# truemeat001/Simple-Raytracing-Render

Measured on AMD Instinct MI355X. Metric: Msamples/s (rays x bounces) + HBM GB/s vs roofline, Cornell+teapot 1024spp, higher is better.
Workload: dtype f32

## Files before the change

### simple-raytracing-render_amd/csrc/capi.cpp

```cpp
#include <hip/hip_runtime.h>

#include <algorithm>
#include <chrono>
#include <cstdint>
#include <cstdio>
#include <cstring>
#include <map>
#include <memory>
#include <string>
#include <vector>

#include "../../include/srr_capi.h"
#include "imageio.h"
#include "meshio.h"
#include "../../include/srr/merl.h"
#include "multi.h"
#include "renderer.h"

using namespace srr;

struct srr_scene {
  Scene s;
};

namespace {
thread_local std::string g_err;

int fail(int code, const std::string& msg) {
  g_err = msg;
  return code;
}

#define HIPCHK(x)                                                                         \
  do {                                                                                    \
    hipError_t e_ = (x);                                                                  \
    if (e_ != hipSuccess) return fail(SRR_EIO, std::string(#x) + ": " + hipGetErrorString(e_)); \
  } while (0)

template <class T>
int upload(T** dst, const std::vector<T>& v) {
  size_t bytes = std::max<size_t>(v.size() * sizeof(T), 16);
  HIPCHK(hipMalloc((void**)dst, bytes));
  if (!v.empty()) HIPCHK(hipMemcpy(*dst, v.data(), v.size() * sizeof(T), hipMemcpyHostToDevice));
  return 0;
}
}

extern "C" {

const char* srr_last_error(void) { return g_err.c_str(); }
const char* srr_version(void) { return "srr 0.1 (gfx950 wavefront path tracer)"; }

srr_scene* srr_scene_create(void) { return new srr_scene(); }
void srr_scene_destroy(srr_scene* s) { delete s; }

int srr_scene_from_text(const char* text, srr_scene** out) {
  if (!text || !out) return fail(SRR_EINVAL, "null argument");
  std::unique_ptr<srr_scene> s(new srr_scene());
  std::string err;
  int rc = scene_from_text(text, s->s, err);
  if (rc < 0) return fail(rc, err);
  *out = s.release();
  return 0;
}

int srr_scene_text_handle(const srr_scene* s, int id) {
  if (!s) return fail(SRR_EINVAL, "null scene");
  for (auto& kv : s->s.text_ids)
    if (kv.first == id) return kv.second;
  return fail(SRR_EINVAL, "no such text object id");
}

int srr_scene_digest(const srr_scene* s, uint64_t* out, uint64_t* parts) {
  if (!s || !out) return fail(SRR_EINVAL, "null argument");
  Flat f;
  std::string err;
  const int rc = flatten(s->s, f, err);
  if (rc < 0) return fail(rc, err);
  uint64_t h = 0xcbf29ce484222325ULL;
  int part = 0;
  auto mix = [](uint64_t& x, const void* p, size_t n) {
    const unsigned char* b = (const unsigned char*)p;
    for (size_t i = 0; i < n; ++i) x = (x ^ b[i]) * 0x100000001b3ULL;
  };
  auto blob = [&](const void* p, size_t n) {
    mix(h, &n, sizeof n);
    mix(h, p, n);
    if (const char* dd = getenv("SRR_DIGEST_DUMP")) {
      FILE* df = fopen((std::string(dd) + "." + std::to_string(part)).c_str(), "wb");
      if (df) { fwrite(p, 1, n, df); fclose(df); }
    }
    if (parts) {
      uint64_t x = 0xcbf29ce484222325ULL;
      mix(x, p, n);
      parts[part] = x;
    }
    ++part;
  };
  auto vec = [&blob](const auto& v) { blob(v.data(), v.size() * sizeof(v[0])); };
  vec(f.objs);
  blob(&f.n_world, sizeof f.n_world);
  vec(f.xforms);
  vec(f.spheres);
  vec(f.rects);
  vec(f.stris);
  vec(f.meshes);
  vec(f.nodes);
  vec(f.node4);
  vec(f.tri_pos);
  vec(f.tri_shade);
  vec(f.media);
  {
    std::vector<uint8_t> b;
    auto put = [&b](const void* p, size_t n) { b.insert(b.end(), (const uint8_t*)p, (const uint8_t*)p + n); };
    put(f.obvhs.data(), f.obvhs.size() * sizeof(DObvh));
    put(f.sgroups.data(), f.sgroups.size() * sizeof(DSGroup));
    put(f.sg_items.data(), f.sg_items.size() * sizeof(DSGItem));
    vec(b);
  }
  vec(f.obvh_children);
  vec(f.mats);
  vec(f.texs);
  vec(f.images);
  vec(f.perlin_ranvec);
  vec(f.perlin_perm);
  vec(f.lights);
  blob(&f.cam, sizeof f.cam);
  *out = h;
  return 0;
}

int srr_scene_set_lcg(srr_scene* s, uint64_t state) {
  if (!s) return fail(SRR_EINVAL, "null scene");
  s->s.lcg = state & 0xFFFFFFFFFFFFULL;
  return 0;
}
uint64_t srr_scene_get_lcg(const srr_scene* s) { return s ? s->s.lcg : 0; }
double srr_scene_drand48(srr_scene* s) { return s ? s->s.drand48() : 0.0; }

#define SCN(s) \
  if (!(s)) return fail(SRR_EINVAL, "null scene");
#define TEXOK(s, t) \
  if (!(s)->s.valid_tex(t)) return fail(SRR_EINVAL, "bad texture handle " + std::to_string(t));
#define MATOK(s, m) \
  if (!(s)->s.valid_mat(m)) return fail(SRR_EINVAL, "bad material handle " + std::to_string(m));
#define OBJOK(s, o) \
  if (!(s)->s.valid_obj(o)) return fail(SRR_EINVAL, "bad hitable handle " + std::to_string(o));

int srr_constant_texture(srr_scene* s, float r, float g, float b) {
  SCN(s);
  HTex t;
  t.kind = TEX_CONST;
  t.c[0] = r; t.c[1] = g; t.c[2] = b;
  return s->s.add_tex(std::move(t));
}
int srr_image_texture(srr_scene* s, const unsigned char* rgb, int nx, int ny) {
  SCN(s);
  if (!rgb || nx <= 0 || ny <= 0) return fail(SRR_EINVAL, "bad image");
  HTex t;
  t.kind = TEX_IMAGE;
  t.nx = nx;
  t.ny = ny;
  t.px.assign(rgb, rgb + (size_t)nx * ny * 3);
  return s->s.add_tex(std::move(t));
}
int srr_image_texture_file(srr_scene* s, const char* path) {
  SCN(s);
  if (!path) return fail(SRR_EINVAL, "null path");
  srr::Image im;
  std::string err;
// ... 301 lines not shown
    hipError_t e = hipMemcpy(h.data(), d, h.size() * sizeof(float), hipMemcpyDeviceToHost);
    if (e != hipSuccess) rc = fail(SRR_EIO, hipGetErrorString(e));
  }
  hipFree(d);
  if (rc < 0) return rc;
  if (mean) std::memcpy(mean, h.data(), h.size() * sizeof(float));
  if (rgb8) srr_tonemap(h.data(), npix, rgb8);
  return 0;
}

int srr_accum_get(srr_renderer* r, float* sums, int64_t* npix, int64_t* samples) {
  if (!r) return fail(SRR_EINVAL, "null renderer");
  if (r && r->multi) return fail(SRR_EINVAL, "progressive sums and kept paths are per device: use a one-device renderer");
  if (npix) *npix = r->acc_npix;
  if (samples) *samples = r->acc_samples;
  if (sums && r->acc_npix) {
    HIPCHK(hipSetDevice(r->device));
    HIPCHK(hipMemcpy(sums, r->acc, 3 * r->acc_npix * sizeof(float), hipMemcpyDeviceToHost));
  }
  return 0;
}

int srr_accum_set(srr_renderer* r, const float* sums, int64_t npix, int64_t samples) {
  if (!r || !sums || npix <= 0 || samples < 0) return fail(SRR_EINVAL, "bad accumulator state");
  if (r && r->multi) return fail(SRR_EINVAL, "progressive sums and kept paths are per device: use a one-device renderer");
  HIPCHK(hipSetDevice(r->device));
  drain_async(r);
  if ((size_t)npix > r->pix_cap) {
    r->pix_key[0] = -1;
    (void)hipFree(r->pixels);
    (void)hipFree(r->acc);
    r->pixels = nullptr;
    r->acc = nullptr;
    r->pix_cap = 0;
    HIPCHK(hipMalloc((void**)&r->pixels, npix * sizeof(int32_t)));
    HIPCHK(hipMalloc((void**)&r->acc, 3 * npix * sizeof(float)));
    r->pix_cap = npix;
  }
  HIPCHK(hipMemcpy(r->acc, sums, 3 * npix * sizeof(float), hipMemcpyHostToDevice));
  r->acc_npix = npix;
  r->acc_samples = samples;
  std::fill(r->acc_key, r->acc_key + 5, -1);
  return 0;
}

int srr_copy_paths(srr_renderer* r, float* radiance, unsigned char* rays) {
  if (r && r->multi) return fail(SRR_EINVAL, "progressive sums and kept paths are per device: use a one-device renderer");
  if (!r || !r->raw_all) return fail(SRR_EINVAL, "render with SRR_FLAG_KEEP_PATHS first");
  HIPCHK(hipSetDevice(r->device));
  if (radiance) HIPCHK(hipMemcpy(radiance, r->raw_all, r->kept_paths * 3 * sizeof(float), hipMemcpyDeviceToHost));
  if (rays) HIPCHK(hipMemcpy(rays, r->rays_all, r->kept_paths, hipMemcpyDeviceToHost));
  return 0;
}

int srr_tonemap(const float* mean, int64_t n, unsigned char* rgb8) {
  if (!mean || !rgb8) return fail(SRR_EINVAL, "null argument");
  for (int64_t i = 0; i < 3 * n; ++i) {
    float c = std::sqrt(mean[i]);
    int q = int(255.99 * c);
    q = q > 255 ? 255 : q;
    q = q < 0 ? 0 : q;
    rgb8[i] = (unsigned char)q;
  }
  return 0;
}

int srr_mesh_file_triangles(const char* path, int flip_uvs, int flip_winding, const float scale[3], float* pos9,
                            float* uv9, float* nrm9, int* flags_out) {
  if (!path || !scale) return fail(SRR_EINVAL, "null argument");
  srr::MeshData m;
  std::string err;
  if (srr::load_mesh_file(path, m, err) < 0) return fail(SRR_EIO, err);
  srr::apply_model_semantics(m, flip_uvs != 0, flip_winding != 0, scale);
  for (size_t t = 0; t < m.tris.size(); ++t)
    for (int j = 0; j < 3; ++j) {
      const srr::MeshData::Corner& c = m.tris[t][j];
      if (pos9) std::memcpy(pos9 + 9 * t + 3 * j, c.p, 12);
      if (uv9) std::memcpy(uv9 + 9 * t + 3 * j, c.uv, 12);
      if (nrm9) std::memcpy(nrm9 + 9 * t + 3 * j, c.n, 12);
    }
  if (flags_out) *flags_out = (m.has_normals ? 1 : 0) | (m.has_uvs ? 2 : 0);
  if (m.tris.size() > (size_t)INT32_MAX / 2) return fail(SRR_EINVAL, "mesh too large");
  return (int)m.tris.size();
}

int srr_model(srr_scene* s, const char* path, int flip_uvs, int flip_winding, int mat, const float scale[3],
              int* first_handle) {
  if (!s || !path || !scale) return fail(SRR_EINVAL, "null argument");
  srr::MeshData m;
  std::string err;
  if (srr::load_mesh_file(path, m, err) < 0) return fail(SRR_EIO, err);
  srr::apply_model_semantics(m, flip_uvs != 0, flip_winding != 0, scale);
  if (m.tris.empty()) return fail(SRR_EINVAL, std::string(path) + ": mesh 0 has no triangles");
  int first = -1;
  for (const auto& t : m.tris) {
    float p[9], uv[9], n[9];
    for (int j = 0; j < 3; ++j) {
      std::memcpy(p + 3 * j, t[j].p, 12);
      std::memcpy(uv + 3 * j, t[j].uv, 12);
      std::memcpy(n + 3 * j, t[j].n, 12);
    }
    int h = srr_triangle(s, p, mat, uv, m.has_normals ? n : nullptr);
    if (h < 0) return h;
    if (first < 0) first = h;
  }
  if (first_handle) *first_handle = first;
  return (int)m.tris.size();
}

int srr_write_ppm(const char* path, int nx, int ny, const unsigned char* rgb8) {
  FILE* f = fopen(path, "w");
  if (!f) return fail(SRR_EIO, std::string("cannot open ") + path);
  fprintf(f, "P3\n%d %d\n255\n", nx, ny);
  for (int i = 0; i < nx * ny; ++i) fprintf(f, "%d %d %d\n", rgb8[3 * i], rgb8[3 * i + 1], rgb8[3 * i + 2]);
  fclose(f);
  return 0;
}

int srr_write_png(const char* path, int nx, int ny, const unsigned char* rgb8) {
  if (!path || !rgb8) return fail(SRR_EINVAL, "null argument");
  std::vector<uint8_t> png;
  std::string err;
  int rc = srr::encode_png(rgb8, nx, ny, 3, png, err);
  if (rc < 0) return fail(rc, err);
  FILE* f = fopen(path, "wb");
  if (!f) return fail(SRR_EIO, std::string("cannot open ") + path);
  size_t w = fwrite(png.data(), 1, png.size(), f);
  fclose(f);
  return w == png.size() ? 0 : fail(SRR_EIO, std::string("short write to ") + path);
}

int srr_image_load(const char* path, int req_comp, int* x, int* y, int* comp, unsigned char** out) {
  if (!path || !x || !y || !out) return fail(SRR_EINVAL, "null argument");
  *out = nullptr;
  srr::Image im;
  std::string err;
  int rc = srr::load_image(path, req_comp, im, err);
  if (rc < 0) return fail(rc == -2 ? SRR_EIO : SRR_EINVAL, err);
  *x = im.w;
  *y = im.h;
  if (comp) *comp = im.file_n;
  *out = (unsigned char*)malloc(im.px.size());
  if (!*out) return fail(SRR_ENOMEM, "out of memory");
  std::memcpy(*out, im.px.data(), im.px.size());
  return im.n;
}

void srr_image_free(unsigned char* pixels) { free(pixels); }

int srr_device_kat(const char* name, int n, int width, float* records) {
  if (!name || !records || n <= 0 || width <= 0) return fail(SRR_EINVAL, "bad KAT arguments");
  static const char* kNames[] = {"erf",   "beckmann11", "beckmann_dist", "beckmann_pdf", "cosine_pdf",
                                 "orennayar_pdf", "dielectric", "metal", "triangle", "aabb", "sqrt",
                                 "camera", "lights", "light_list"};
  static const int kWidth[] = {3, 5, 16, 21, 21, 21, 14, 14, 26, 15, 2, 23, 15, 15};
  int kind = -1;
  for (int k = 0; k < 14; ++k)
    if (!strcmp(name, kNames[k])) kind = k;
  if (kind < 0) return fail(SRR_EINVAL, std::string("no device KAT named ") + name);
  if (width != kWidth[kind]) return fail(SRR_EINVAL, std::string("KAT ") + name + ": unexpected record width");
  std::vector<float> aux(4 * (size_t)n, 0.f);
  std::vector<DStandaloneTri> tris(kind == 8 ? n : 1);
  Scene hs;
  for (int q = 0; q < n; ++q) {
    const float* r = records + (size_t)q * width;
    if (kind == 2 || kind == 3) {
      const float prm[4] = {r[0], r[1], 0, 0};
      const HMat& m = hs.mat[hs.material(MAT_BECKMANN, -1, prm)];
      aux[4 * q] = m.p[0];
      aux[4 * q + 1] = m.p[1];
    } else if (kind == 4 || kind == 5) {
      const float prm[4] = {r[0], 0, 0, 0};
      const HMat& m = hs.mat[hs.material(MAT_ORENNAYAR, -1, prm)];
      aux[4 * q] = m.p[0];
      aux[4 * q + 1] = m.p[1];
    } else if (kind == 8) {
      const float uv9[9] = {0.1f, 0.2f, 0, 0.7f, 0.1f, 0, 0.3f, 0.9f, 0};
      const int h = hs.triangle(r, -1, uv9, nullptr);
      const HTri& t = hs.tris[hs.obj[h].tri];
      DStandaloneTri& d = tris[q];
      std::memcpy(d.p, t.p, 36);
      std::memcpy(d.sh.n, t.n, 36);
      for (int k = 0; k < 3; ++k) d.sh.uv[2 * k] = t.uv[3 * k], d.sh.uv[2 * k + 1] = t.uv[3 * k + 1];
      d.sh.mat = -1;
    }
  }
  std::vector<DCamera> cams(kind == 11 ? n : 1);
  if (kind == 11) {
    for (int q = 0; q < n; ++q) {
      const float* r = records + (size_t)q * width;
      const float vup[3] = {0, 1, 0};
      Scene cs;
      cs.camera(r, r + 3, vup, r[6], r[7], r[8], r[9], 0.0f, 1.0f);
      const HCamera& c = cs.cam;
      DCamera& d = cams[q];
      std::memcpy(d.origin, c.origin, 12);
      std::memcpy(d.llc, c.llc, 12);
      std::memcpy(d.horizontal, c.horizontal, 12);
      std::memcpy(d.vertical, c.vertical, 12);
      std::memcpy(d.u, c.u, 12);
      std::memcpy(d.v, c.v, 12);
      d.time0 = c.time0;
      d.time1 = c.time1;
      d.lens_radius = c.lens_radius;
    }
  }
  Flat lf;
  if (kind == 12 || kind == 13) {
    Scene ls;
    const int rect = ls.wrap(H_FLIP, ls.rect(H_XZ, 213, 343, 227, 332, 554, -1), nullptr);
    const float c[3] = {278, 700, 280};
    const int sph = ls.sphere(c, 50, -1);
    const float p9[9] = {150, 500, 150, 400, 520, 180, 260, 540, 420};
    const int tri = ls.triangle(p9, -1, nullptr, nullptr);
    const int kids[3] = {rect, sph, tri};
    ls.world = ls.lights = ls.list(kids, 3);
    const float lf3[3] = {0, 0, -1}, la3[3] = {0, 0, 0}, up[3] = {0, 1, 0};
    ls.camera(lf3, la3, up, 40, 1, 0, 1, 0, 1);
    ls.has_camera = true;
    std::string e;
    if (flatten(ls, lf, e) < 0 || lf.lights.size() != 3) return fail(SRR_EINVAL, "light KAT scene: " + e);
  }
  float* d_rec = nullptr;
  float* d_aux = nullptr;
  DStandaloneTri* d_tris = nullptr;
  DCamera* d_cams = nullptr;
  DRect* d_rects = nullptr;
  DSphere* d_sph = nullptr;
  DStandaloneTri* d_stris = nullptr;
  DLight* d_lights = nullptr;
  const size_t rb = (size_t)n * width * sizeof(float);
  int rc = 0;
  if (hipMalloc((void**)&d_rec, rb) != hipSuccess || hipMalloc((void**)&d_aux, aux.size() * 4) != hipSuccess ||
      hipMalloc((void**)&d_tris, tris.size() * sizeof(DStandaloneTri)) != hipSuccess)
    rc = fail(SRR_ENOMEM, "device allocation failed");
  if (!rc && (hipMemcpy(d_rec, records, rb, hipMemcpyHostToDevice) != hipSuccess ||
              hipMemcpy(d_aux, aux.data(), aux.size() * 4, hipMemcpyHostToDevice) != hipSuccess ||
              hipMemcpy(d_tris, tris.data(), tris.size() * sizeof(DStandaloneTri), hipMemcpyHostToDevice) != hipSuccess))
    rc = fail(SRR_EIO, "copy to device failed");
  auto upload = [&rc](auto*& dst, const auto& v) {
    if (rc || v.empty()) return;
    const size_t b = v.size() * sizeof(v[0]);
    if (hipMalloc((void**)&dst, b) != hipSuccess) rc = fail(SRR_ENOMEM, "device allocation failed");
    else if (hipMemcpy(dst, v.data(), b, hipMemcpyHostToDevice) != hipSuccess) rc = fail(SRR_EIO, "copy to device failed");
  };
  upload(d_cams, cams);
  upload(d_rects, lf.rects);
  upload(d_sph, lf.spheres);
  upload(d_stris, lf.stris);
  upload(d_lights, lf.lights);
  const KatTables kt{d_cams, d_rects, d_sph, d_stris, d_lights, (int)lf.lights.size()};
  if (!rc && launch_kat(kind, n, width, d_rec, d_aux, d_tris, kt) < 0) rc = fail(SRR_EIO, "KAT kernel launch failed");
  if (!rc && (hipDeviceSynchronize() != hipSuccess || hipMemcpy(records, d_rec, rb, hipMemcpyDeviceToHost) != hipSuccess))
    rc = fail(SRR_EIO, "KAT kernel failed");
  for (void* p : {(void*)d_rec, (void*)d_aux, (void*)d_tris, (void*)d_cams, (void*)d_rects, (void*)d_sph,
                  (void*)d_stris, (void*)d_lights})
    (void)hipFree(p);
  return rc;
}

struct srr_merl {
  int device = 0;
  double* table = nullptr;
};

int srr_merl_create(const double* table, int64_t n_doubles, int device, srr_merl** out) {
  if (!table || !out) return fail(SRR_EINVAL, "null argument");
  if (n_doubles != 3 * (int64_t)merl::kCells) return fail(SRR_EINVAL, "MERL table: dimensions don't match");
  HIPCHK(hipSetDevice(device));
  auto m = std::make_unique<srr_merl>();
  m->device = device;
  HIPCHK(hipMalloc((void**)&m->table, (size_t)n_doubles * sizeof(double)));
  if (hipMemcpy(m->table, table, (size_t)n_doubles * sizeof(double), hipMemcpyHostToDevice) != hipSuccess) {
    (void)hipFree(m->table);
    return fail(SRR_EIO, "MERL table upload failed");
  }
  *out = m.release();
  return 0;
}

int srr_merl_load(const char* path, int device, srr_merl** out) {
  if (!path || !out) return fail(SRR_EINVAL, "null argument");
  FILE* f = fopen(path, "rb");
  if (!f) return fail(SRR_EIO, std::string("cannot open MERL table ") + path);
  int32_t dims[3] = {0, 0, 0};
  const bool hdr = fread(dims, sizeof(int32_t), 3, f) == 3;
  const int64_t n = (int64_t)dims[0] * dims[1] * dims[2];
  if (!hdr || n != merl::kCells) {
    fclose(f);
    return fail(SRR_EINVAL, "MERL table: dimensions don't match");
  }
  std::vector<double> t(3 * (size_t)n);
  const size_t got = fread(t.data(), sizeof(double), t.size(), f);
  fclose(f);
  if (got != t.size()) return fail(SRR_EINVAL, "MERL table: truncated file");
  return srr_merl_create(t.data(), (int64_t)t.size(), device, out);
}

void srr_merl_destroy(srr_merl* m) {
  if (!m) return;
  (void)hipSetDevice(m->device);
  (void)hipFree(m->table);
  delete m;
}

int srr_merl_lookup(srr_merl* m, int64_t n, const double* angles, double* rgb, int32_t* cell) {
  if (!m || n < 0 || (n > 0 && (!angles || !rgb))) return fail(SRR_EINVAL, "bad MERL lookup arguments");
  if (n == 0) return 0;
  HIPCHK(hipSetDevice(m->device));
  double *d_ang = nullptr, *d_rgb = nullptr;
  int32_t* d_cell = nullptr;
  int rc = 0;
  if (hipMalloc((void**)&d_ang, 4 * (size_t)n * sizeof(double)) != hipSuccess ||
      hipMalloc((void**)&d_rgb, 3 * (size_t)n * sizeof(double)) != hipSuccess ||
      (cell && hipMalloc((void**)&d_cell, (size_t)n * sizeof(int32_t)) != hipSuccess))
    rc = fail(SRR_ENOMEM, "device allocation failed");
  if (!rc && hipMemcpy(d_ang, angles, 4 * (size_t)n * sizeof(double), hipMemcpyHostToDevice) != hipSuccess)
    rc = fail(SRR_EIO, "copy to device failed");
  if (!rc && launch_merl_lookup(m->table, n, d_ang, d_rgb, d_cell) < 0) rc = fail(SRR_EIO, "MERL kernel launch failed");
  if (!rc && (hipDeviceSynchronize() != hipSuccess ||
              hipMemcpy(rgb, d_rgb, 3 * (size_t)n * sizeof(double), hipMemcpyDeviceToHost) != hipSuccess ||
              (cell && hipMemcpy(cell, d_cell, (size_t)n * sizeof(int32_t), hipMemcpyDeviceToHost) != hipSuccess)))
    rc = fail(SRR_EIO, "MERL kernel failed");
  (void)hipFree(d_ang);
  (void)hipFree(d_rgb);
  (void)hipFree(d_cell);
  return rc;
}

int srr_teapot_vertices(float scale, int divs, float* out) {
  if (divs < 1 || divs > 400) return fail(SRR_EINVAL, "teapot divs out of range");
  std::vector<float> p;
  teapot_triangles(scale, divs, p);
  if (out) std::memcpy(out, p.data(), p.size() * sizeof(float));
  return (int)(p.size() / 9);
}

int64_t srr_bvh_topology(const srr_scene* s, int o, char* buf, int64_t cap) {
  if (!s || !s->s.valid_obj(o) || s->s.obj[o].kind != H_BVH) return fail(SRR_EINVAL, "not a bvh_node handle");
  const HBvh& B = s->s.bvhs[s->s.obj[o].bvh];
  std::map<int, int> pos;
  for (size_t q = 0; q < B.input.size(); ++q) pos[B.input[q]] = (int)q;
  std::string txt;
  char line[256];
  snprintf(line, sizeof line, "box %g %g %g %g %g %g\n", B.box.mn[0], B.box.mn[1], B.box.mn[2], B.box.mx[0],
           B.box.mx[1], B.box.mx[2]);
  txt += line;
  std::vector<int> stack{0};
  while (!stack.empty()) {
    int n = stack.back();
    stack.pop_back();
    const HBvh::Node& nd = B.nodes[n];
    if (nd.left < 0) {
      snprintf(line, sizeof line, "L %d %d\n", pos[B.leaves[~nd.left]], pos[B.leaves[~nd.right]]);
      txt += line;
    } else {
      txt += "N\n";
      stack.push_back(nd.right);
      stack.push_back(nd.left);
    }
  }
  if (buf && cap > 0) {
    int64_t m = std::min<int64_t>(cap - 1, (int64_t)txt.size());
    std::memcpy(buf, txt.data(), m);
    buf[m] = 0;
  }
  return (int64_t)txt.size() + 1;
}

int srr_sobol_points(int n, double* out) {
  if (n < 1 || !out) return fail(SRR_EINVAL, "bad args");
  sobol2((unsigned)n, out);
  return 0;
}

}
```

### simple-raytracing-render_amd/csrc/device_scene.h

```cpp
#pragma once
#include <cstdint>

namespace srr {

enum ObjKind : int32_t {
  OBJ_SPHERE = 0,
  OBJ_MSPHERE = 1,
  OBJ_RECT = 2,
  OBJ_TRI = 3,
  OBJ_MESH = 4,
  OBJ_MEDIUM = 5,
  OBJ_OBVH = 6,
  OBJ_SGROUP = 7,
};

enum XformKind : int32_t { XF_FLIP = 0, XF_TRANSLATE = 1, XF_ROTY = 2, XF_ROTX = 3 };

struct DXform {
  int32_t kind;
  float a, b, c;
};

constexpr int32_t kXfFlipBit = 1 << 30;
constexpr int32_t kXfCountMask = 0xFFFF;

struct DObj {
  int32_t kind;
  int32_t xf_begin, xf_count;
  int32_t idx;
};

struct DSphere {
  float c0[3], c1[3];
  float t0, t1, r;
  int32_t mat;
};

struct DRect {
  int32_t kax, a0, a1, mat;
  float lo0, hi0, lo1, hi1, k;
  float pad[3];
};

struct TriShade {
  float n[9];
  float uv[6];
  int32_t mat;
};

constexpr int kNode4qWords = 16;

struct DMesh {
  int32_t node_off;
  int32_t tri_off;
  int32_t n_nodes, n_tris;
  int32_t node4_off;
  int32_t n_node4;
};

struct DObvh {
  int32_t node_off, n_nodes;
  int32_t child_off, n_children;
};

struct DObvhChild {
  int32_t obj_begin, obj_count;
};

constexpr int kSGroupMinRun = 8;

struct DSGroup {
  int32_t node_off, n_nodes;
  int32_t item_off, n_items;
};

struct DSGItem {
  DSphere s;
  int32_t pos;
  int32_t moving;
  int32_t obj;
  int32_t pad;
};

struct DMedium {
  int32_t bnd_begin, bnd_count;
  float density;
  int32_t phase_mat;
};

enum MatKind : int32_t {
  MAT_LAMBERTIAN = 0,
  MAT_ORENNAYAR = 1,
  MAT_BECKMANN = 2,
  MAT_METAL = 3,
  MAT_DIELECTRIC = 4,
  MAT_DIFFUSE_LIGHT = 5,
  MAT_ISOTROPIC = 6,
  MAT_COUNT = 7,
};

struct DMat {
  int32_t kind;
  int32_t tex;
  float p[4];
};

enum TexKind : int32_t { TEX_CONST = 0, TEX_IMAGE = 1, TEX_CHECKER = 2, TEX_NOISE = 3 };

struct DTex {
  int32_t kind;
  int32_t nx, ny;
  int32_t even, odd;
  int64_t off;
  float c[3];
};

enum LightKind : int32_t { LIGHT_NONE = 0, LIGHT_XZRECT = 1, LIGHT_SPHERE = 2, LIGHT_TRI = 3 };

struct DLight {
  int32_t kind;
  int32_t idx;
};

struct DCamera {
  float origin[3], llc[3], horizontal[3], vertical[3], u[3], v[3];
  float time0, time1, lens_radius;
};

struct DStandaloneTri {
  float p[9];
  TriShade sh;
};

}
```

### simple-raytracing-render_amd/csrc/kernels.h

```cpp
#pragma once
#include <hip/hip_runtime.h>

#include <cstdint>

#include "device_scene.h"

namespace srr {

struct SceneView {
  const DObj* objs;
  int n_world;
  int has_media;
  const DXform* xforms;
  const DSphere* spheres;
  const DRect* rects;
  const DStandaloneTri* stris;
  const DMesh* meshes;
  const float4* nodes;
  const float4* node4;
  int node4_lds;
  int node4_total;
  const float4* node4q;
  int node4_lds_q;
  int use_q;
  int quad_trace;
  int quad_max;
  int mesh_obj;
  const float4* tri_pos;
  const float4* tri_edge;
  const TriShade* tri_shade;
  const DMedium* media;
  const DObvh* obvhs;
  const DObvhChild* obvh_children;
  const DSGroup* sgroups;
  const DSGItem* sg_items;
  const DMat* mats;
  const DTex* texs;
  const uint8_t* images;
  const float* perlin_ranvec;
  const int32_t* perlin_perm;
  const DLight* lights;
  int n_lights;
  float light_weight;
  const DCamera* cam;
  const uint4* world_blob;
  int world_words;
  int world_off[10];
};

struct PathState {
  float4* ray_o;
  float4* ray_d;
  uint64_t* lcg;
  uint64_t* pcg;
  int32_t* depth;
  uint64_t* spec;
  int4* hit_w;
  float4* hit_p;
  float4* hit_n;
  float4* rec_a;
  float* sample;
  float* raw;
  uint8_t* rays;
};

struct BatchInfo {
  int32_t* active;
  int32_t* count;
  int act0;
  int slot0;
  const int32_t* pixels;
  const double* sobol;
  int p0;
  int n_paths;
  int s0, spp_batch;
  int s_base;
  int nx, ny;
  uint64_t base_seed;
};

struct UDiv31 {
  uint32_t m, p;
};
inline UDiv31 make_udiv31(uint32_t d) {
  uint32_t l = 0;
  while ((1ull << l) < d) ++l;
  const uint32_t p = 31 + l;
  return UDiv31{(uint32_t)(((1ull << p) + d - 1) / d), p};
}

struct PathWork {
  const int32_t* pixels;
  const double* sobol;
  int npix, spp_w;
  int s_base;
  int nx, ny;
  UDiv31 div_spp, div_nx;
  uint64_t base_seed;
  int64_t n_paths;
  int max_depth;
  unsigned long long* cursor;
  unsigned long long* counters;
  float* sample;
  float* raw;
  uint8_t* rays;
  int keep_spp, keep_s0;
  float4* rec;
  int lanes;
  int* err;
  int stack_cap;
  int2* gstack;
  int gstack_cap;
  unsigned long long* wave_times;
  int deep_tries;
  float* slow_rays;
  unsigned* slow_count;
  int walk_q;
};
#ifndef SRR_KSTACK
#define SRR_KSTACK 8
#endif
constexpr int kPathsLdsStack = SRR_KSTACK;
constexpr int kPathsGlobalStack = 56;

constexpr int kPathsWorldLdsBytes = 8192;
#ifndef SRR_LDS_NODES
#define SRR_LDS_NODES 96
#endif
constexpr int kPathsLdsNodes = SRR_LDS_NODES;
void dump_trace_timing();
int paths_lanes_per_device(const SceneView& S, int device);
int paths_block_lanes(const SceneView& S);
int launch_paths(const SceneView& S, const PathWork& W, int all_families, hipStream_t st);
struct KatTables {
  const DCamera* cams;
  const DRect* rects;
  const DSphere* spheres;
  const DStandaloneTri* stris;
  const DLight* lights;
  int n_lights;
};
int launch_kat(int kind, int n, int w, float* d_rec, const float* d_aux, const DStandaloneTri* d_tris,
               const KatTables& kt);
int launch_merl_lookup(const double* table, int64_t n, const double* angles, double* rgb, int32_t* cell);
void launch_accumulate_window(const float* sample, int npix, int spp_w, float* acc, hipStream_t st, bool init = false,
                              float* out = nullptr, int scale_ns = 0);
void launch_raygen(const SceneView& S, const PathState& P, const BatchInfo& B, hipStream_t st);
void launch_trace(const SceneView& S, const PathState& P, const int* active, const int* count, int max_n,
                  int* lists, int list_cap, int* fam_count, int* fetch, int max_depth, unsigned long long* ctr,
                  hipStream_t st);
void launch_shade(const SceneView& S, const PathState& P, const int* lists, int list_cap, const int* fam_count,
                  int* next, int* next_count, int* region_alive, int region_size, int max_n, int max_depth,
                  hipStream_t st);
void launch_accumulate(const PathState& P, const BatchInfo& B, float* acc, hipStream_t st);
void launch_finish(const float* acc, float* mean, int64_t n, int ns, hipStream_t st);
void launch_scatter_pixels(const float* packed, const int32_t* index, int64_t n, float* image, hipStream_t st);

}
```

### simple-raytracing-render_amd/csrc/kernels.hip

```cpp
#include <hip/hip_runtime.h>

#include <cfloat>
#include <algorithm>
#include <cstdint>
#include <cstdlib>
#include <cstring>

#include "device_scene.h"
#include "devmath.h"
#include "kernels.h"
#include "../../include/srr/merl.h"

namespace srr {
namespace dev {

SRR_D V3 sphere_center(const DSphere& s, float tm, bool moving) {
  V3 c0 = v3(s.c0[0], s.c0[1], s.c0[2]);
  if (!moving) return c0;
  V3 c1 = v3(s.c1[0], s.c1[1], s.c1[2]);
  return c0 + ((tm - s.t0) / (s.t1 - s.t0)) * (c1 - c0);
}

SRR_D bool sphere_hit(const DSphere& s, bool moving, const Ray& r, float tmin, float tmax, float& t) {
  V3 oc = r.o - sphere_center(s, r.tm, moving);
  float a = dot(r.d, r.d);
  float b = dot(oc, r.d);
  float c = dot(oc, oc) - s.r * s.r;
  float disc = b * b - a * c;
  if (disc > 0) {
    float sq = rsqrt_exact(disc);
    float temp = (-b - sq) / a;
    if (temp < tmax && temp > tmin) { t = temp; return true; }
    temp = (-b + sq) / a;
    if (temp < tmax && temp > tmin) { t = temp; return true; }
  }
  return false;
}

template <int KAX>
SRR_D bool rect_hit_t(const DRect& q, const Ray& r, float tmin, float tmax, float& t) {
  constexpr int A0 = KAX == 0 ? 1 : 0, A1 = KAX == 2 ? 1 : 2;
  const float tt = (q.k - r.o[KAX]) / r.d[KAX];
  if (tt < tmin || tt > tmax) return false;
  const float x = r.o[A0] + tt * r.d[A0];
  const float y = r.o[A1] + tt * r.d[A1];
  if (x < q.lo0 || x > q.hi0 || y < q.lo1 || y > q.hi1) return false;
  t = tt;
  return true;
}

#ifndef SRR_RECTAX
#define SRR_RECTAX 1
#endif
SRR_D bool rect_hit(const DRect& q, const Ray& r, float tmin, float tmax, float& t, float& u, float& v) {
#ifdef SRR_EXP_FASTRECT
  float tt = (q.k - r.o[q.kax]) * __builtin_amdgcn_rcpf(r.d[q.kax]);
#else
  float tt = (q.k - r.o[q.kax]) / r.d[q.kax];
#endif
  if (tt < tmin || tt > tmax) return false;
  float x = r.o[q.a0] + tt * r.d[q.a0];
  float y = r.o[q.a1] + tt * r.d[q.a1];
  if (x < q.lo0 || x > q.hi0 || y < q.lo1 || y > q.hi1) return false;
  u = (x - q.lo0) / (q.hi0 - q.lo0);
  v = (y - q.lo1) / (q.hi1 - q.lo1);
  t = tt;
  return true;
}

SRR_D bool tri_hit(V3 p0, V3 p1, V3 p2, bool front, V3 o, V3 dir, float& t, float& u, float& v) {
  V3 e1, e2;
  if (front) { e1 = p1 - p0; e2 = p2 - p0; }
  else { e1 = p0 - p1; e2 = p2 - p1; }
  V3 P = cross(dir, e2);
  float det = dot(e1, P);
  V3 T;
  if (det > 0) T = o - p0;
  else { T = p0 - o; det = -det; }
  if (det < kUp1em4) return false;
  float uu = dot(T, P);
  if (uu < 0.0f || uu > det) return false;
  V3 Q = cross(T, e1);
  float vv = dot(dir, Q);
  if (vv < 0.0f || vv + uu > det) return false;
  float tt = dot(e2, Q);
  float inv = 1.0f / det;
  tt *= inv;
  uu *= inv;
  vv *= inv;
  if (tt < kUp1em4) return false;
  t = tt; u = uu; v = vv;
  return true;
}

SRR_D bool tri_hit_e(V3 p0, V3 e1, V3 e2, V3 o, V3 dir, float& t) {
  V3 P = cross(dir, e2);
  float det = dot(e1, P);
  V3 T;
  if (det > 0) T = o - p0;
  else { T = p0 - o; det = -det; }
  if (det < kUp1em4) return false;
  float uu = dot(T, P);
  if (uu < 0.0f || uu > det) return false;
  V3 Q = cross(T, e1);
  float vv = dot(dir, Q);
  if (vv < 0.0f || vv + uu > det) return false;
  float tt = dot(e2, Q);
  float inv = 1.0f / det;
  tt *= inv;
  if (tt < kUp1em4) return false;
  t = tt;
  return true;
}

constexpr int kTriStride = 4;

SRR_D bool slab(float4 lo, float4 hi, V3 o, V3 inv, float tmin, float tmax) {
#define SRR_AX(A)                                     \
  {                                                   \
    float t0 = (lo.A - o.A) * inv.A;                  \
    float t1 = (hi.A - o.A) * inv.A;                  \
    bool sw = inv.A < 0.0f;                           \
    float n_ = sw ? t1 : t0, f_ = sw ? t0 : t1;       \
    tmin = n_ > tmin ? n_ : tmin;                     \
    tmax = f_ < tmax ? f_ : tmax;                     \
  }
  SRR_AX(x) SRR_AX(y) SRR_AX(z)
#undef SRR_AX
  return !(tmax <= tmin);
}

struct MeshHit {
  float t;
  int tri;
};

SRR_D bool wins(float t, int ti, float best_t, int best_i) {
  return ti > best_i ? !(best_t < t) : (t < best_t);
}

template <bool PREFETCH>
SRR_D bool mesh_hit(const SceneView& S, const DMesh& m, const Ray& r, float tmin, float tmax, bool is_medium,
                    MeshHit& out, unsigned long long* ctr) {
  V3 inv = v3(1.0f / r.d.x, 1.0f / r.d.y, 1.0f / r.d.z);
  V3 dir = r.d / length(r.d);
  int node = m.node_off;
  const int end = m.node_off + m.n_nodes;
  bool found = false;
  float best_t = 0;
  int best_i = -1;
  uint32_t nbox = 0, ntri = 0;
  float4 lo = S.nodes[2 * (node)], hi = S.nodes[2 * (node) + 1];
  for (;;) {
    ++nbox;
    const int skip = __float_as_int(lo.w);
    const int leaf = __float_as_int(hi.w);
    float4 lo_c, hi_c, lo_s, hi_s;
    if (PREFETCH) {
      if (leaf < 0) { lo_c = S.nodes[2 * (node + 1)]; hi_c = S.nodes[2 * (node + 1) + 1]; }
      if (skip < end) { lo_s = S.nodes[2 * (skip)]; hi_s = S.nodes[2 * (skip) + 1]; }
    }
    bool hit = slab(lo, hi, r.o, inv, tmin, tmax);
    if (hit && leaf >= 0) {
      int first = leaf >> 1, count = (leaf & 1) + 1;
      ntri += 2;
      for (int ti = first; ti < first + count; ++ti) {
        const float4* tp = S.tri_pos + kTriStride * (size_t)ti;
        float4 a = tp[0], b = tp[1], c = tp[2];
        V3 p0 = v3(a.x, a.y, a.z), p1 = v3(b.x, b.y, b.z), p2 = v3(c.x, c.y, c.z);
        float t, u, v;
        bool h = tri_hit(p0, p1, p2, true, r.o, dir, t, u, v);
        if (!h && is_medium) { ++ntri; h = tri_hit(p0, p1, p2, false, r.o, dir, t, u, v); }
        if (h && (!found || wins(t, ti, best_t, best_i))) {
          found = true;
          best_t = t;
          best_i = ti;
        }
      }
    }
    const bool down = hit && leaf < 0;
    const int next = down ? node + 1 : skip;
    if (next >= end) break;
    if (PREFETCH) {
      lo = down ? lo_c : lo_s;
      hi = down ? hi_c : hi_s;
    } else {
      lo = S.nodes[2 * (next)];
      hi = S.nodes[2 * (next) + 1];
    }
    node = next;
  }
  if (ctr) { atomicAdd(ctr, (unsigned long long)nbox); atomicAdd(ctr + 1, (unsigned long long)ntri); }
  out.t = best_t;
// ... 1302 lines not shown
#pragma unroll
          for (int k = 0; k < 25; ++k) t[k] = q[k];
        } else {
          T = S.stris[ob.idx];
        }
        p0 = v3(T.p[0], T.p[1], T.p[2]);
        p1 = v3(T.p[3], T.p[4], T.p[5]);
        p2 = v3(T.p[6], T.p[7], T.p[8]);
        shv = T.sh;
      } else {
        const float4* tp = S.tri_pos + kTriStride * (size_t)prim;
        float4 a = tp[0], b = tp[1], c = tp[2];
        p0 = v3(a.x, a.y, a.z);
        p1 = v3(b.x, b.y, b.z);
        p2 = v3(c.x, c.y, c.z);
        shv = S.tri_shade[prim];
      }
      const TriShade* sh = &shv;
      V3 dir = lr.d / length(lr.d);
      float tt, u, v;
      tri_hit(p0, p1, p2, true, lr.o, dir, tt, u, v);
      float a0 = 1 - u - v;
      float uvx = a0 * sh->uv[0] + u * sh->uv[2] + v * sh->uv[4];
      float uvy = a0 * sh->uv[1] + u * sh->uv[3] + v * sh->uv[5];
      h.u = uvx;
      h.v = uvy;
      V3 n0 = v3(sh->n[0], sh->n[1], sh->n[2]), n1 = v3(sh->n[3], sh->n[4], sh->n[5]),
         n2 = v3(sh->n[6], sh->n[7], sh->n[8]);
      h.n = unit_vector(a0 * n0 + u * n1 + v * n2);
      h.p = a0 * p0 + u * p1 + v * p2;
      h.mat = sh->mat;
      break;
    }
    case OBJ_MEDIUM: {
      h.p = lr.at(t);
      h.n = v3(1, 0, 0);
      h.mat = S.media[ob.idx].phase_mat;
      break;
    }
  }
}

template <int TR = 0>
SRR_D HitRec world_record(const SceneView& S, const Ray& r, const WorldHit& w) {
  const DObj& ob = S.objs[w.obj];
  Ray lr = chain_in<TR>(S, ob, r);
  HitRec h;
  h.u = 0;
  h.v = 0;
  if (ob.kind == OBJ_OBVH || ob.kind == OBJ_SGROUP) {
    const DObj& in = S.objs[ob.kind == OBJ_SGROUP ? S.sg_items[w.prim].obj : w.prim];
    prim_record<TR>(S, in, chain_in<TR>(S, in, lr), w.t, -1, h);
    chain_out(S, in, h.p, h.n);
  } else {
    prim_record<TR>(S, ob, lr, w.t, w.prim, h);
  }
  chain_out(S, ob, h.p, h.n);
  return h;
}

enum Family : int { FAM_TERM = 0, FAM_DIFF = 1, FAM_BECK = 2, FAM_SPEC = 3 };

SRR_D int family_of(int mat, int kind, int depth, int max_depth) {
  if (mat < 0 || kind == MAT_DIFFUSE_LIGHT || depth >= max_depth) return FAM_TERM;
  if (kind == MAT_LAMBERTIAN || kind == MAT_ORENNAYAR) return FAM_DIFF;
  if (kind == MAT_BECKMANN) return FAM_BECK;
  return FAM_SPEC;
}

SRR_D int hit_material(const SceneView& S, const WorldHit& w) {
  DObj ob = S.objs[w.obj];
  if (ob.kind == OBJ_OBVH) ob = S.objs[w.prim];
  else if (ob.kind == OBJ_SGROUP) ob = S.objs[S.sg_items[w.prim].obj];
  switch (ob.kind) {
    case OBJ_SPHERE:
    case OBJ_MSPHERE: return S.spheres[ob.idx].mat;
    case OBJ_RECT: return S.rects[ob.idx].mat;
    case OBJ_TRI: return S.stris[ob.idx].sh.mat;
    case OBJ_MESH: return S.tri_shade[w.prim].mat;
    case OBJ_MEDIUM: return S.media[ob.idx].phase_mat;
  }
  return -1;
}

SRR_D void store_hit(const SceneView& S, const PathState& P, int p, const WorldHit& w, int max_depth, int& fam) {
  if (w.obj < 0) {
    nts(&P.hit_w[p], make_int4(-1, -1, 0, -1));
    fam = FAM_TERM;
    return;
  }
  const int mat = hit_material(S, w);
  nts(&P.hit_w[p], make_int4(w.obj, w.prim, __float_as_int(w.t), mat));
  fam = family_of(mat, mat >= 0 ? S.mats[mat].kind : -1, ntl(&P.depth[p]), max_depth);
}

constexpr int kMixtureGuard = 100000;
SRR_D V3 tex_value_slow(const SceneView& S, int ti, float u, float v, V3 p) {
  for (int guard = 0; guard < 8; ++guard) {
    const DTex& T = S.texs[ti];
    if (T.kind == TEX_CONST) return v3(T.c[0], T.c[1], T.c[2]);
    if (T.kind == TEX_IMAGE) {
      int i = (u) * T.nx;
      int j = (1 - v) * T.ny - 0.001;
      if (i < 0) i = 0;
      if (j < 0) j = 0;
      if (i > T.nx - 1) i = T.nx - 1;
      if (j > T.ny - 1) j = T.ny - 1;
      const uint8_t* px = S.images + T.off + 3 * (size_t)i + 3 * (size_t)T.nx * j;
      float r = (float)int(px[0]) / 255.0f;
      float g = (float)int(px[1]) / 255.0f;
      float b = (float)int(px[2]) / 255.0f;
      return v3(r, g, b);
    }
    if (T.kind == TEX_CHECKER) {
      float sines = rsin(10 * p.x) * rsin(10 * p.y) * rsin(10 * p.z);
      ti = sines < 0 ? T.odd : T.even;
      continue;
    }
    float scale = T.c[0];
    V3 tp = scale * p;
    float accum = 0, weight = 1.0f;
    for (int oct = 0; oct < 7; ++oct) {
      float fx = floorf(tp.x), fy = floorf(tp.y), fz = floorf(tp.z);
      float uu = tp.x - fx, vv = tp.y - fy, ww = tp.z - fz;
      int i = (int)fx, j = (int)fy, k = (int)fz;
      float hu = uu * uu * (3 - 2 * uu), hv = vv * vv * (3 - 2 * vv), hw = ww * ww * (3 - 2 * ww);
      float acc = 0;
      for (int a = 0; a < 2; a++)
        for (int b = 0; b < 2; b++)
          for (int c = 0; c < 2; c++) {
            int idx = S.perlin_perm[(i + a) & 255] ^ S.perlin_perm[256 + ((j + b) & 255)] ^
                      S.perlin_perm[512 + ((k + c) & 255)];
            V3 g = v3(S.perlin_ranvec[3 * idx], S.perlin_ranvec[3 * idx + 1], S.perlin_ranvec[3 * idx + 2]);
            V3 wv = v3(uu - a, vv - b, ww - c);
            acc += (a * hu + (1 - a) * (1 - hu)) * (b * hv + (1 - b) * (1 - hv)) * (c * hw + (1 - c) * (1 - hw)) *
                   dot(g, wv);
          }
      accum += weight * acc;
      weight *= 0.5f;
      tp = tp * 2.0f;
    }
    float turb = fabsf(accum);
    return v3(1, 1, 1) * 0.5f * (1 + rsin(scale * p.z + 5 * turb));
  }
  return v3(0.f);
}

SRR_D V3 tex_value(const SceneView& S, int ti, float u, float v, V3 p) {
  const DTex& T = S.texs[ti];
  if (T.kind == TEX_CONST) return v3(T.c[0], T.c[1], T.c[2]);
  return tex_value_slow(S, ti, u, v, p);
}

struct Onb {
  V3 u, v, w;
};
SRR_D Onb onb_from_w(V3 n) {
  Onb o;
  o.w = unit_vector(n);
  V3 a = (fabsf(o.w.x) >= kUp0p9) ? v3(0, 1, 0) : v3(1, 0, 0);
  o.v = unit_vector(cross(o.w, a));
  o.u = cross(o.w, o.v);
  return o;
}
SRR_D V3 onb_local(const Onb& b, V3 a) { return a.x * b.u + a.y * b.v + a.z * b.w; }

SRR_D float Cos2Theta(V3 w) { return w.z * w.z; }
SRR_D float AbsCosTheta(V3 w) { return fabsf(w.z); }
SRR_D float Sin2Theta(V3 w) { return fmaxf(0.0f, 1.0f - Cos2Theta(w)); }
SRR_D float SinTheta(V3 w) { return rsqrt_exact(Sin2Theta(w)); }
SRR_D float TanTheta(V3 w) { return SinTheta(w) / w.z; }
SRR_D float Tan2Theta(V3 w) { return Sin2Theta(w) / Cos2Theta(w); }
SRR_D float clamp11(float x) { return x < -1 ? -1.f : (x > 1 ? 1.f : x); }
SRR_D float CosPhi(V3 w) {
  float s = SinTheta(w);
  return (s == 0) ? 1 : clamp11(w.x / s);
}
SRR_D float SinPhi(V3 w) {
  float s = SinTheta(w);
  return (s == 0) ? 0 : clamp11(w.y / s);
}
SRR_D float Cos2Phi(V3 w) { return CosPhi(w) * CosPhi(w); }
SRR_D float Sin2Phi(V3 w) { return SinPhi(w) * SinPhi(w); }

SRR_D float Erf(float x) {
  float a1 = 0.254829592f, a2 = -0.284496736f, a3 = 1.421413741f, a4 = -1.453152027f, a5 = 1.061405429f;
  float p = 0.3275911f;
  int sign = 1;
  if (x < 0) sign = -1;
  x = fabsf(x);
  float t = 1 / (1 + p * x);
  float y = 1 - (((((a5 * t + a4) * t) + a3) * t + a2) * t + a1) * t + rexp(-x * x);
  return sign * y;
}
SRR_D float ErfInv(float x) {
  float w, p;
  x = x < -.99999f ? -.99999f : (x > .99999f ? .99999f : x);
  w = -rlog((1 - x) * (1 + x));
  if (w < 5) {
    w = w - 2.5f;
    p = 2.81022636e-08f;
    p = 3.43273939e-07f + p * w;
    p = -3.5233877e-06f + p * w;
    p = -4.39150654e-06f + p * w;
    p = 0.00021858087f + p * w;
    p = -0.00125372503f + p * w;
    p = -0.00417768164f + p * w;
    p = 0.246640727f + p * w;
    p = 1.50140941f + p * w;
  } else {
    w = rsqrt_exact(w) - 3;
    p = -0.000200214257f;
    p = 0.000100950558f + p * w;
    p = 0.00134934322f + p * w;
    p = -0.00367342844f + p * w;
    p = 0.00573950773f + p * w;
    p = -0.0076224613f + p * w;
    p = 0.00943887047f + p * w;
    p = 1.00167406f + p * w;
    p = 2.83297682f + p * w;
  }
  return p * x;
}

struct Beck {
  float ax, ay;
  SRR_D float D(V3 wh) const {
    float tan2 = Tan2Theta(wh);
    if (isinf(tan2)) return 0.;
    float cos4 = Cos2Theta(wh) * Cos2Theta(wh);
    return rexp(-tan2 * (Cos2Phi(wh) / (ax * ax) + Sin2Phi(wh) / (ay * ay))) / (kPi * ax * ay * cos4);
  }
  SRR_D float Lambda(V3 w) const {
    float absTan = fabsf(TanTheta(w));
    if (isinf(absTan)) return 0;
    float alpha = rsqrt_exact(Cos2Phi(w) * ax * ax + Sin2Phi(w) * ay * ay);
    float a = 1 / (alpha * absTan);
    if (a > 1.6f) return 0;
    return (1 - 1.259f * a + 0.396f * a * a) / (3.535f * a + 2.181f * a * a);
  }
  SRR_D float G1(V3 w) const { return 1 / (1 + Lambda(w)); }
  SRR_D float G(V3 wo, V3 wi) const { return 1 / (1 + Lambda(wo) + Lambda(wi)); }
  SRR_D float Pdf(V3 wo, V3 wh) const { return D(wh) * G1(wo) * fabsf(dot(wo, wh)) / AbsCosTheta(wo); }
};

SRR_D void beckmann_sample11(float cosThetaI, float u1, float u2, float& sx, float& sy) {
  if (cosThetaI > .9999) {
    float r = rsqrt_exact(-rlog(1.0f - u1));
    float sinPhi = ::sin(2 * kPi * u2);
    float cosPhi = ::cos(2 * kPi * u2);
    sx = r * cosPhi;
    sy = r * sinPhi;
    return;
  }
  float sinThetaI = rsqrt_exact(fmaxf(0.0f, 1.0f - cosThetaI * cosThetaI));
  float tanThetaI = sinThetaI / cosThetaI;
  float cotThetaI = 1 / tanThetaI;
  float a = -1, c = Erf(cosThetaI);
  float sample_x = fmaxf(u1, 1e-6f);
  float thetaI = racos(cosThetaI);
  float fit = 1 + thetaI * (-0.876f + thetaI * (0.4265f - 0.0594f * thetaI));
  float b = c - (1 + c) * rpow(1 - sample_x, fit);
  const float SQRT_PI_INV = (float)(1.f / ::sqrt(kPi));
  float normalization = 1 / (1 + c + SQRT_PI_INV * tanThetaI * rexp(-cotThetaI * cotThetaI));
  int it = 0;
  float invErf = 0;
  bool fresh = false;
  while (++it < 10) {
    if (!(b >= a && b <= c)) b = 0.5f * (a + c);
    invErf = ErfInv(b);
    float value = normalization * (1 + b + SQRT_PI_INV * tanThetaI * (rexp(-invErf * invErf))) - sample_x;
    float derivative = normalization * (1 - invErf * tanThetaI);
    if (fabsf(value) < 1e-5f) {
      fresh = true;
      break;
    }
    if (value > 0) c = b;
    else a = b;
    b -= value / derivative;
  }
  sx = fresh ? invErf : ErfInv(b);
  sy = ErfInv(2.0f * fmaxf(u2, 1e-6f) - 1.0f);
}

SRR_D V3 beckmann_sample_wh(const Beck& d, V3 wo, float u1, float u2) {
  bool flip = wo.z < 0;
  V3 wi = flip ? -wo : wo;
  V3 ws = unit_vector(v3(d.ax * wi.x, d.ay * wi.y, wi.z));
  float sx, sy;
  beckmann_sample11(ws.z, u1, u2, sx, sy);
  float tmp = CosPhi(ws) * sx - SinPhi(ws) * sy;
  sy = SinPhi(ws) * sx + CosPhi(ws) * sy;
  sx = tmp;
  sx = d.ax * sx;
  sy = d.ay * sy;
  V3 wh = unit_vector(v3(-sx, -sy, 1.f));
  if (flip) wh = -wh;
  return wh;
}

struct BeckPre {
  V3 wwo;
  V3 uw;
  float cphi, sphi;
  float ct;
  float tan_t, c, fit, norm;
  float lam1;
  bool flip;
};

SRR_D void beckmann_pre(const Beck& d, const Onb& uvw, V3 wo, BeckPre& p) {
  const V3 mwo = -wo;
  p.wwo = unit_vector(v3(dot(mwo, uvw.u), dot(mwo, uvw.v), dot(mwo, uvw.w)));
  p.uw = unit_vector(p.wwo);
  p.flip = p.wwo.z < 0;
  const V3 wi = p.flip ? -p.wwo : p.wwo;
  const V3 ws = unit_vector(v3(d.ax * wi.x, d.ay * wi.y, wi.z));
  p.cphi = CosPhi(ws);
  p.sphi = SinPhi(ws);
  p.ct = ws.z;
  p.tan_t = p.c = p.fit = p.norm = 0;
  if (!(p.ct > .9999)) {
    const float cosThetaI = p.ct;
    float sinThetaI = rsqrt_exact(fmaxf(0.0f, 1.0f - cosThetaI * cosThetaI));
    float tanThetaI = sinThetaI / cosThetaI;
    float cotThetaI = 1 / tanThetaI;
    p.c = Erf(cosThetaI);
    float thetaI = racos(cosThetaI);
    p.fit = 1 + thetaI * (-0.876f + thetaI * (0.4265f - 0.0594f * thetaI));
    const float SQRT_PI_INV = (float)(1.f / ::sqrt(kPi));
    p.norm = 1 / (1 + p.c + SQRT_PI_INV * tanThetaI * rexp(-cotThetaI * cotThetaI));
    p.tan_t = tanThetaI;
  }
  p.lam1 = 1 + d.Lambda(wo);
}

SRR_D void beckmann_sample11_pre(const BeckPre& p, float u1, float u2, float& sx, float& sy) {
  if (p.ct > .9999) {
    float r = rsqrt_exact(-rlog(1.0f - u1));
    float sinPhi = ::sin(2 * kPi * u2);
    float cosPhi = ::cos(2 * kPi * u2);
    sx = r * cosPhi;
    sy = r * sinPhi;
    return;
  }
  const float tanThetaI = p.tan_t, normalization = p.norm;
  float a = -1, c = p.c;
  float sample_x = fmaxf(u1, 1e-6f);
  float b = c - (1 + c) * rpow(1 - sample_x, p.fit);
  const float SQRT_PI_INV = (float)(1.f / ::sqrt(kPi));
  int it = 0;
  float invErf = 0;
  bool fresh = false;
  while (++it < 10) {
    if (!(b >= a && b <= c)) b = 0.5f * (a + c);
    invErf = ErfInv(b);
    float value = normalization * (1 + b + SQRT_PI_INV * tanThetaI * (rexp(-invErf * invErf))) - sample_x;
    float derivative = normalization * (1 - invErf * tanThetaI);
    if (fabsf(value) < 1e-5f) {
      fresh = true;
      break;
    }
    if (value > 0) c = b;
    else a = b;
    b -= value / derivative;
  }
  sx = fresh ? invErf : ErfInv(b);
  sy = ErfInv(2.0f * fmaxf(u2, 1e-6f) - 1.0f);
}

SRR_D V3 beckmann_sample_wh_pre(const Beck& d, const BeckPre& p, float u1, float u2) {
  float sx, sy;
  beckmann_sample11_pre(p, u1, u2, sx, sy);
  float tmp = p.cphi * sx - p.sphi * sy;
  sy = p.sphi * sx + p.cphi * sy;
  sx = tmp;
  sx = d.ax * sx;
  sy = d.ay * sy;
  V3 wh = unit_vector(v3(-sx, -sy, 1.f));
  if (p.flip) wh = -wh;
  return wh;
}

#ifndef SRR_SINCOS
#define SRR_SINCOS 1
#endif
SRR_D V3 random_cosine_direction(Rng& rng) {
  float r1 = drand(rng);
  float r2 = drand(rng);
  float phi = 2 * kPi * r1;
  float z = rsqrt_exact(1 - r2);
#if SRR_SINCOS && !defined(SRR_LIBM_DOUBLE)
  float sp, cp;
  gm::sincosf_(phi, sp, cp);
  float x = cp * 2 * rsqrt_exact(r2);
  float y = sp * 2 * rsqrt_exact(r2);
#else
  float x = rcos(phi) * 2 * rsqrt_exact(r2);
  float y = rsin(phi) * 2 * rsqrt_exact(r2);
#endif
  return v3(x, y, z);
}

SRR_D V3 random_in_unit_sphere(Rng& rng) {
  V3 p;
  do {
    float z = (float)drand(rng);
    float y = (float)drand(rng);
    float x = (float)drand(rng);
    p = 2.0f * v3(x, y, z) - v3(1, 1, 1);
  } while (dot(p, p) >= 1.0);
  return p;
}

__device__ __noinline__ float light_pdf_other(const DSphere* spheres, const DStandaloneTri* stris, DLight L, V3 o,
                                              V3 v);

SRR_D float light_pdf_one(const SceneView& S, const DLight& L, V3 o, V3 v) {
  Ray r{o, v, 0.0f};
  if (L.kind == LIGHT_XZRECT) {
    const DRect& q = S.rects[L.idx];
    float t;
#if SRR_RECTAX
    if (rect_hit_t<1>(q, r, 0.001f, FLT_MAX, t)) {
#else
    float u, vv;
    if (rect_hit(q, r, 0.001f, FLT_MAX, t, u, vv)) {
#endif
      float area = (q.hi0 - q.lo0) * (q.hi1 - q.lo1);
      float distance_square = t * t * squared_length(v);
      float cosine = fabsf(v.y / length(v));
      return distance_square / (cosine * area);
    }
    return 0;
  }
  if (L.kind == LIGHT_NONE) return 0.0;
  return light_pdf_other(S.spheres, S.stris, L, o, v);
}

__device__ __noinline__ float light_pdf_other(const DSphere* spheres, const DStandaloneTri* stris, DLight L, V3 o,
                                              V3 v) {
  Ray r{o, v, 0.0f};
  if (L.kind == LIGHT_SPHERE) {
    const DSphere& s = spheres[L.idx];
    float t;
    if (sphere_hit(s, false, r, 0.001f, FLT_MAX, t)) {
      V3 c = v3(s.c0[0], s.c0[1], s.c0[2]);
      float cos_theta_max = rsqrt_exact(1 - s.r * s.r / squared_length(c - o));
      float solid_angle = 2 * kPi * (1 - cos_theta_max);
      return 1 / solid_angle;
    }
    return 0;
  }
  if (L.kind == LIGHT_TRI) {
    const DStandaloneTri& T = stris[L.idx];
    V3 p0 = v3(T.p[0], T.p[1], T.p[2]), p1 = v3(T.p[3], T.p[4], T.p[5]), p2 = v3(T.p[6], T.p[7], T.p[8]);
    float t, u, vv;
    if (tri_hit(p0, p1, p2, true, o, v / length(v), t, u, vv)) {
      const TriShade& sh = T.sh;
      float a0 = 1 - u - vv;
      V3 n = unit_vector(a0 * v3(sh.n[0], sh.n[1], sh.n[2]) + u * v3(sh.n[3], sh.n[4], sh.n[5]) +
                         vv * v3(sh.n[6], sh.n[7], sh.n[8]));
      V3 v01 = p1 - p0;
      V3 v01n = v01 / length(v01);
      V3 v02 = p2 - p0;
      V3 v02n = v02 / length(v02);
      float cos102 = dot(v01n, v02n);
      float sin102 = rsqrt_exact(1 - cos102 * cos102);
      float h = length(v02) * sin102;
      float area = 0.5 * length(v01) * h;
      float distance_square = t * t * squared_length(v);
      float cosine = fabsf(dot(v, n)) / length(v);
      return distance_square / (cosine * area);
    }
    return 0;
  }
  return 0.0;
}

SRR_D float lights_pdf(const SceneView& S, V3 o, V3 v) {
  const float weight = S.light_weight;
  float sum = 0;
  for (int k = 0; k < S.n_lights; ++k) sum += weight * light_pdf_one(S, S.lights[k], o, v);
  return sum;
}

struct LightDraw {
  V3 d;
  uint64_t lcg;
};
__device__ __noinline__ LightDraw light_random_other(const DSphere* spheres, const DStandaloneTri* stris, DLight L,
                                                     V3 o, uint64_t lcg);

SRR_D V3 light_random_one(const SceneView& S, const DLight& L, V3 o, Rng& rng) {
  if (L.kind == LIGHT_XZRECT) {
    const DRect& q = S.rects[L.idx];
    float z = q.lo1 + drand(rng) * (q.hi1 - q.lo1);
    float x = q.lo0 + drand(rng) * (q.hi0 - q.lo0);
    return v3(x, q.k, z) - o;
  }
  if (L.kind == LIGHT_NONE) return v3(1, 0, 0);
  const LightDraw ld = light_random_other(S.spheres, S.stris, L, o, rng.lcg);
  rng.lcg = ld.lcg;
  return ld.d;
}

SRR_D V3 lights_random(const SceneView& S, V3 o, Rng& rng) {
  int index = int(drand(rng) * S.n_lights);
  return light_random_one(S, S.lights[index], o, rng);
}

__device__ __noinline__ LightDraw light_random_other(const DSphere* spheres, const DStandaloneTri* stris, DLight L,
                                                     V3 o, uint64_t lcg) {
  Rng rng{lcg, 0};
  if (L.kind == LIGHT_SPHERE) {
    const DSphere& s = spheres[L.idx];
    V3 dirc = v3(s.c0[0], s.c0[1], s.c0[2]) - o;
    float d2 = squared_length(dirc);
    Onb uvw = onb_from_w(dirc);
    float r1 = drand(rng);
    float r2 = drand(rng);
    float z = 1 + r2 * (rsqrt_exact(1 - s.r * s.r / d2) - 1);
    float phi = 2 * kPi * r1;
    float x = rcos(phi) * rsqrt_exact(1 - z * z);
    float y = rsin(phi) * rsqrt_exact(1 - z * z);
    return LightDraw{onb_local(uvw, v3(x, y, z)), rng.lcg};
  }
  if (L.kind == LIGHT_TRI) {
    const DStandaloneTri& T = stris[L.idx];
    float u = drand(rng);
    float v = drand(rng) * (1 - u);
    V3 p0 = v3(T.p[0], T.p[1], T.p[2]), p1 = v3(T.p[3], T.p[4], T.p[5]), p2 = v3(T.p[6], T.p[7], T.p[8]);
    return LightDraw{p0 * (1 - u - v) + p1 * u + p2 * v - o, rng.lcg};
  }
  return LightDraw{v3(1, 0, 0), rng.lcg};
}

struct Bsdf {
  int kind;
  Onb uvw;
  V3 n;
  float A, B;
  Beck dist;
  float beck_pdf;
  float co;
  V3 lo;
  bool flip;
  BeckPre bp;
};

SRR_D V3 to_local_unit(const Onb& b, V3 d) {
  V3 ud = unit_vector(d);
  return unit_vector(v3(dot(ud, b.u), dot(ud, b.v), dot(ud, b.w)));
}

template <bool BECK>
SRR_D V3 bsdf_generate(Bsdf& f, V3 wo, Rng& rng) {
  if (BECK) {
    (void)wo;
    float u1 = pcg_uniform(rng);
    float u2 = pcg_uniform(rng);
    const BeckPre& p = f.bp;
    V3 wh = beckmann_sample_wh_pre(f.dist, p, u1, u2);
    V3 wi = -p.uw + 2 * dot(p.uw, wh) * wh;
    V3 wwi = unit_vector(wi.x * f.uvw.u + wi.y * f.uvw.v + wi.z * f.uvw.w);
    f.beck_pdf = f.dist.D(wh) * (1 / (p.lam1 + f.dist.Lambda(wi))) / (4 * AbsCosTheta(wi) * AbsCosTheta(p.wwo));
    if (!(wi.z * p.wwo.z > 0)) f.beck_pdf = 0;
    return wwi;
  }
  V3 g = random_cosine_direction(rng);
  if (f.flip) g.z *= -1;
  return onb_local(f.uvw, g);
}

template <bool BECK>
SRR_D void bsdf_prepare(Bsdf& f, V3 wo) {
  if (BECK) {
    beckmann_pre(f.dist, f.uvw, wo, f.bp);
    return;
  }
  f.flip = dot(-wo, f.n) > 0;
  float co = 0;
  V3 lo = v3(0.f);
  if (f.kind == MAT_LAMBERTIAN) co = dot(unit_vector(wo), f.n);
  else lo = to_local_unit(f.uvw, -wo);
  f.co = co;
  f.lo = lo;
}

template <bool BECK>
SRR_D float bsdf_value(const Bsdf& f, V3 wo, V3 wi) {
  (void)wo;
  if (BECK) return f.beck_pdf;
  if (f.kind == MAT_LAMBERTIAN) {
    const float co = f.co;
    float ci = dot(unit_vector(wi), f.n);
    if (ci * co < 0) return fabsf(ci) / kPi;
    return 0;
  }
  const V3 lo = f.lo;
  V3 li = to_local_unit(f.uvw, wi);
  float sinThetaI = SinTheta(li), sinThetaO = SinTheta(lo);
  float maxCos = 0;
  if (sinThetaI > 1e-4 && sinThetaO > 1e-4) {
    float sinPhiI = SinPhi(li), cosPhiI = CosPhi(li);
    float sinPhiO = SinPhi(lo), cosPhiO = CosPhi(lo);
    float dCos = cosPhiI * cosPhiO + sinPhiI * sinPhiO;
    maxCos = ffmax(0.0f, dCos);
  }
  float sinAlpha, tanBeta;
  if (AbsCosTheta(li) > AbsCosTheta(lo)) {
    sinAlpha = sinThetaO;
    tanBeta = sinThetaI / AbsCosTheta(li);
  } else {
    sinAlpha = sinThetaI;
    tanBeta = sinThetaO / AbsCosTheta(lo);
  }
  float cosine = li.z;
  if (cosine < 0) cosine = 0;
  return cosine * (f.A + f.B * maxCos * sinAlpha * tanBeta) / kPi;
}

template <bool BECK>
SRR_D float scattering_pdf(const Bsdf& f, V3 n, V3 rin, V3 sc) {
  if (BECK) {
    V3 wo = to_local_unit(f.uvw, -rin);
    V3 wi = to_local_unit(f.uvw, sc);
    V3 wh = unit_vector(wi + wo);
    return f.dist.Pdf(wo, wh) / (4 * dot(wo, wh));
  }
  float c = dot(n, unit_vector(sc));
  if (c < 0) c = 0;
  return c / kPi;
}

__device__ __forceinline__ int lane_id() { return __lane_id(); }

__device__ __forceinline__ void append(bool pred, int value, int* list, int* count) {
  uint64_t mask = __ballot(pred);
  if (!mask) return;
  int leader = __ffsll((unsigned long long)mask) - 1;
  int base = 0;
  if (lane_id() == leader) base = atomicAdd(count, __popcll(mask));
  base = __shfl(base, leader);
  if (pred) {
    int rank = __popcll(mask & ((1ull << lane_id()) - 1));
    list[base + rank] = value;
  }
}

__device__ __forceinline__ void append4(int fam, int value, int* lists, int list_cap, int* counts) {
  const uint64_t m0 = __ballot(fam == 0), m1 = __ballot(fam == 1), m2 = __ballot(fam == 2), m3 = __ballot(fam == 3);
  if ((m0 | m1 | m2 | m3) == 0) return;
  const int l = lane_id();
  const uint64_t mine = l == 0 ? m0 : l == 1 ? m1 : l == 2 ? m2 : m3;
  int base = 0;
  if (l < 4 && mine) base = atomicAdd(counts + l, __popcll(mine));
  base = __shfl(base, fam >= 0 ? fam : 0);
  if (fam >= 0) {
    const uint64_t m = fam == 0 ? m0 : fam == 1 ? m1 : fam == 2 ? m2 : m3;
    lists[fam * list_cap + base + __popcll(m & ((1ull << l) - 1))] = value;
  }
}


struct DiffSetup {
  V3 p;
  V3 w, v;
  V3 nl;
  float c0, c1;
  int flags;
};

SRR_D DiffSetup diff_setup(const Bsdf& f, V3 p) {
  const bool on = f.kind != MAT_LAMBERTIAN;
  V3 nl = f.n;
  float c0 = f.co;
  if (on) {
    nl = f.lo;
    c0 = f.A;
  }
  return DiffSetup{p, f.uvw.w, f.uvw.v, nl, c0, f.B, (on ? 1 : 0) | (f.flip ? 2 : 0)};
}

SRR_D Bsdf bsdf_of(const DiffSetup& d) {
  Bsdf f;
  f.kind = (d.flags & 1) ? (int)MAT_ORENNAYAR : (int)MAT_LAMBERTIAN;
  f.uvw.w = d.w;
  f.uvw.v = d.v;
  f.uvw.u = cross(d.w, d.v);
  f.n = d.nl;
  f.lo = d.nl;
  f.co = d.c0;
  f.A = d.c0;
  f.B = d.c1;
  f.flip = (d.flags & 2) != 0;
  return f;
}

SRR_D float mixture_attempt(const SceneView& S, Bsdf& f, V3 hpt, Rng& rng, V3& ndir) {
  if (drand(rng) < 0.5) ndir = lights_random(S, hpt, rng);
  else ndir = bsdf_generate<false>(f, v3(0.f), rng);
  return 0.5 * lights_pdf(S, hpt, ndir) + 0.5 * bsdf_value<false>(f, v3(0.f), ndir);
}

SRR_D uint64_t lcg_step(uint64_t s) { return (0x5DEECE66DULL * s + 0xB16ULL) & 0xFFFFFFFFFFFFULL; }

SRR_D uint64_t skip_attempt(const SceneView& S, uint64_t s) {
  s = lcg_step(s);
  if ((s >> 47) == 0) {
    s = lcg_step(s);
    const int idx = int((double)(uint32_t)(s >> 16) / 4294967296.0 * S.n_lights);
    if (S.lights[idx].kind != LIGHT_NONE) s = lcg_step(lcg_step(s));
  } else {
    s = lcg_step(lcg_step(s));
  }
  return s;
}


#ifndef SRR_COOP_HELPERS
#define SRR_COOP_HELPERS 8
#endif
#ifndef SRR_COOP_ID0
#define SRR_COOP_ID0 0
#endif
constexpr int kMaxHelpers = SRR_COOP_HELPERS;

SRR_D int coop_mixture(const SceneView& S, const DiffSetup& me, bool& pend, int& tries, uint64_t& lcg, V3& ndir,
                       float& pdf, int deep_tries) {
  int rounds = 0;
  const int lane = lane_id();
  const uint64_t lt = (1ull << lane) - 1;
  uint64_t F = __ballot(pend);
  bool first = SRR_COOP_ID0 != 0;
  while (F) {
    const int nF = __popcll(F);
    const int cap = __ballot(pend && tries < deep_tries) == 0 ? 64 : kMaxHelpers;
    const int rank = pend ? __popcll(F & lt) : nF + __popcll(~F & lt);
    DiffSetup d;
    int t0, k;
    uint64_t s;
    if (first) {
      d = me;
      t0 = tries;
      s = lcg;
      k = pend ? 0 : 64;
    } else {
      const int owner_of = __builtin_amdgcn_ds_permute(rank << 2, lane);
      const int q = lane % nF;
      k = lane / nF;
      const int src = __builtin_amdgcn_ds_bpermute(q << 2, owner_of);
      d.p = v3(__shfl(me.p.x, src), __shfl(me.p.y, src), __shfl(me.p.z, src));
      d.w = v3(__shfl(me.w.x, src), __shfl(me.w.y, src), __shfl(me.w.z, src));
      d.v = v3(__shfl(me.v.x, src), __shfl(me.v.y, src), __shfl(me.v.z, src));
      d.nl = v3(__shfl(me.nl.x, src), __shfl(me.nl.y, src), __shfl(me.nl.z, src));
      d.c0 = __shfl(me.c0, src);
      d.c1 = __shfl(me.c1, src);
      d.flags = __shfl(me.flags, src);
      t0 = __shfl(tries, src);
      s = ((uint64_t)(uint32_t)__shfl((int)(uint32_t)(lcg >> 32), src) << 32) |
          (uint32_t)__shfl((int)(uint32_t)lcg, src);
    }
    const bool active = k < cap && t0 + k < kMixtureGuard;
    V3 nd = v3(0.f);
    float pv = 0;
    if (active) {
      for (int j = 0; j < k; ++j) s = skip_attempt(S, s);
      Rng rr{s, 0};
      Bsdf f = bsdf_of(d);
      pv = mixture_attempt(S, f, d.p, rr, nd);
      s = rr.lcg;
    }
    const uint64_t ok = __ballot(active && (pv != 0 || t0 + k + 1 >= kMixtureGuard));
    if (first) {
      if (pend) {
        lcg = s;
        if ((ok >> lane) & 1) {
          ndir = nd;
          pdf = pv;
          pend = false;
        } else {
          tries += 1;
        }
      }
      first = false;
    } else {
      int win = lane, m = 0;
      if (pend) {
        m = min(cap, (63 - rank) / nF + 1);
        m = min(m, kMixtureGuard - tries);
        int j = 0;
        while (j < m - 1 && !((ok >> (rank + j * nF)) & 1)) ++j;
        win = rank + j * nF;
      }
      const float wx = __shfl(nd.x, win), wy = __shfl(nd.y, win), wz = __shfl(nd.z, win), wp = __shfl(pv, win);
      const uint64_t ws = ((uint64_t)(uint32_t)__shfl((int)(uint32_t)(s >> 32), win) << 32) |
                          (uint32_t)__shfl((int)(uint32_t)s, win);
      if (pend) {
        lcg = ws;
        if ((ok >> win) & 1) {
          ndir = v3(wx, wy, wz);
          pdf = wp;
          pend = false;
        } else {
          tries += m;
        }
      }
    }
    F = __ballot(pend);
    ++rounds;
  }
  return rounds;
}

SRR_D void camera_get_ray(const DCamera& C, float u, float v, Rng& rng, V3& o, V3& dir, float& time) {
  V3 pd;
  do {
    float y = drand(rng);
    float x = drand(rng);
    pd = 2.0f * v3(x, y, 0) - v3(1, 1, 0);
  } while (dot(pd, pd) >= 1.0);
  V3 rd = C.lens_radius * pd;
  V3 cu = v3(C.u[0], C.u[1], C.u[2]), cv = v3(C.v[0], C.v[1], C.v[2]);
  V3 offset = cu * rd.x + cv * rd.y;
  time = C.time0 + drand(rng) * (C.time1 - C.time0);
  V3 org = v3(C.origin[0], C.origin[1], C.origin[2]);
  dir = v3(C.llc[0], C.llc[1], C.llc[2]) + u * v3(C.horizontal[0], C.horizontal[1], C.horizontal[2]) +
        v * v3(C.vertical[0], C.vertical[1], C.vertical[2]) - org - offset;
  dir = unit_vector(dir);
  o = org + offset;
}

#ifndef SRR_MIXTURE_SKIP
#define SRR_MIXTURE_SKIP 2
#endif

SRR_D bool light_point_far(V3 c, V3 p, V3 w, float sgn, float m) { return sgn * dot(c - p, w) <= -m; }

SRR_D bool bsdf_dead(const SceneView& S, const Bsdf& f, V3 p) {
  if (f.kind == MAT_LAMBERTIAN) {
    if (f.flip ? !(f.co <= 0) : !(f.co >= 0)) return false;
  } else if (!f.flip) {
    return false;
  }
  const float sgn = f.flip ? -1.f : 1.f;
  const V3 w = f.uvw.w;
  const float ps = fmaxf(fmaxf(fabsf(p.x), fabsf(p.y)), fabsf(p.z)) + 1.f;
  for (int k = 0; k < S.n_lights; ++k) {
    const DLight L = S.lights[k];
    if (L.kind == LIGHT_XZRECT) {
      const DRect q = S.rects[L.idx];
#if SRR_XFAX
      if (!(q.k != p.y)) return false;
#else
      if (!(q.k != p[q.kax])) return false;
#endif
      const float m = 1e-3f * (ps + fmaxf(fmaxf(fmaxf(fabsf(q.lo0), fabsf(q.hi0)), fmaxf(fabsf(q.lo1), fabsf(q.hi1))),
                                          fabsf(q.k)));
      for (int c = 0; c < 4; ++c) {
#if SRR_XFAX
        const V3 v = v3((c & 1) ? q.hi0 : q.lo0, q.k, (c & 2) ? q.hi1 : q.lo1);
#else
        V3 v = v3(0.f);
        v.set(q.kax, q.k);
        v.set(q.a0, (c & 1) ? q.hi0 : q.lo0);
        v.set(q.a1, (c & 2) ? q.hi1 : q.lo1);
#endif
        if (!light_point_far(v, p, w, sgn, m)) return false;
      }
    } else if (L.kind == LIGHT_SPHERE) {
      const DSphere sp = S.spheres[L.idx];
      const V3 c = v3(sp.c0[0], sp.c0[1], sp.c0[2]);
      const float r = fabsf(sp.r);
      const float m = 1e-3f * (ps + fmaxf(fmaxf(fabsf(c.x), fabsf(c.y)), fabsf(c.z)) + r);
      if (!light_point_far(c, p, w, sgn, r + m)) return false;
    } else if (L.kind == LIGHT_TRI) {
      const DStandaloneTri& T = S.stris[L.idx];
      float cs = 0;
#pragma unroll
      for (int k2 = 0; k2 < 9; ++k2) cs = fmaxf(cs, fabsf(T.p[k2]));
      const float m = 1e-3f * (ps + cs);
#pragma unroll
      for (int c = 0; c < 3; ++c)
        if (!light_point_far(v3(T.p[3 * c], T.p[3 * c + 1], T.p[3 * c + 2]), p, w, sgn, m)) return false;
    } else if (L.kind != LIGHT_NONE) {
      return false;
    }
  }
  return true;
}

SRR_D int skip_mixture(const SceneView& S, const DiffSetup& me, bool dead, bool& pend, int& tries, uint64_t& lcg,
                       V3& ndir, float& pdf, int max_rounds = 1 << 30) {
  int rounds = 0;
  while (rounds < max_rounds && __ballot(pend)) {
    if (pend) {
      uint64_t s = lcg;
      int t = tries;
      if (dead) {
        while (t + 1 < kMixtureGuard) {
          const uint64_t s1 = lcg_step(s);
          if ((s1 >> 47) == 0) break;
          const uint64_t s3 = lcg_step(lcg_step(s1));
          const float r2 = (float)((double)(uint32_t)(s3 >> 16) / 4294967296.0);
          if (!(r2 <= 0.999f)) break;
          s = s3;
          ++t;
        }
      }
      Rng rr{s, 0};
      Bsdf f = bsdf_of(me);
      V3 nd;
      const float pv = mixture_attempt(S, f, me.p, rr, nd);
      lcg = rr.lcg;
      tries = t + 1;
      if (pv != 0 || tries >= kMixtureGuard) {
        ndir = nd;
        pdf = pv;
        pend = false;
      }
    }
    ++rounds;
  }
  return rounds;
}

SRR_D void sobol2_point(uint32_t i, double& sx, double& sy) {
  const uint32_t g = i ^ (i >> 1);
  uint32_t y = 0, v = 0x80000000u;
  for (uint32_t t = g; t; t >>= 1, v ^= v >> 1)
    if (t & 1) y ^= v;
  sx = (double)__builtin_bitreverse32(g) / 4294967296.0;
  sy = (double)y / 4294967296.0;
}

SRR_D uint32_t udiv31(uint32_t n, UDiv31 v) { return (uint32_t)(((uint64_t)n * v.m) >> v.p); }

SRR_D void camera_ray(const SceneView& S, int pix, int s_global, double sx, double sy, int nx, int ny,
                      uint64_t base_seed, V3& o, V3& dir, float& time, Rng& rng, const UDiv31* dnx = nullptr) {
  const int q = dnx ? (int)udiv31((uint32_t)pix, *dnx) : pix / nx;
  int i = pix - q * nx;
  int j = ny - 1 - q;
  uint64_t h = 0xcbf29ce484222325ULL ^ base_seed;
  uint32_t w[3] = {(uint32_t)i, (uint32_t)j, (uint32_t)s_global};
#pragma unroll
  for (int k = 0; k < 3; ++k)
#pragma unroll
    for (int b = 0; b < 4; ++b) {
      h ^= (w[k] >> (8 * b)) & 0xffu;
      h *= 0x100000001b3ULL;
    }
  rng.lcg = h & 0xFFFFFFFFFFFFULL;
  rng.pcg = 0x853c49e6748fea9bULL ^ (rng.lcg << 16);
  float u = float(sx + i) / float(nx);
  float v = float(sy + j) / float(ny);
  camera_get_ray(*S.cam, u, v, rng, o, dir, time);
}


__global__ void __launch_bounds__(256) k_raygen(SceneView S, PathState P, BatchInfo B) {
  int q = blockIdx.x * blockDim.x + threadIdx.x;
  if (q >= B.n_paths) return;
  int lp = q / B.spp_batch;
  int s = B.s0 + q % B.spp_batch;
  int p = B.slot0 + q;
  if (q == 0) *B.count = B.act0 + B.n_paths;
  int pix = B.pixels[B.p0 + lp];
  Rng rng;
  V3 o, dir;
  float time;
  camera_ray(S, pix, B.s_base + s, B.sobol[2 * s], B.sobol[2 * s + 1], B.nx, B.ny, B.base_seed, o, dir, time, rng);
  nts(&P.ray_o[p], make_float4(o.x, o.y, o.z, time));
  nts(&P.ray_d[p], make_float4(dir.x, dir.y, dir.z, 0.f));
  nts(&P.lcg[p], rng.lcg);
  nts(&P.pcg[p], rng.pcg);
  nts(&P.depth[p], 0);
  nts(&P.spec[p], 0);
  B.active[B.act0 + q] = p;
  if (P.rays) P.rays[p] = 0;
}


template <bool MEDIA, int TR>
__global__ void __launch_bounds__(kTraceBlock) k_trace(SceneView S0, PathState P, const int* active, const int* count,
                                                       int* lists, int list_cap, int* fam_count, int max_depth,
                                                       unsigned long long* ctr) {
  const uint64_t t_start = tr_mode(TR) == TR_BVH4_TIMED ? __builtin_amdgcn_s_memtime() : 0;
  SceneView S = S0;
  if constexpr ((TR & TR_WL) != 0) {
    __shared__ uint4 s_world[kWorldLdsBytes / 16];
    for (int i = threadIdx.x; i < S0.world_words; i += blockDim.x) s_world[i] = S0.world_blob[i];
    __syncthreads();
    const char* b = (const char*)s_world;
    S.objs = (const DObj*)(b + S0.world_off[0]);
    S.xforms = (const DXform*)(b + S0.world_off[1]);
    S.spheres = (const DSphere*)(b + S0.world_off[2]);
    S.rects = (const DRect*)(b + S0.world_off[3]);
    S.stris = (const DStandaloneTri*)(b + S0.world_off[4]);
    S.meshes = (const DMesh*)(b + S0.world_off[5]);
    S.media = (const DMedium*)(b + S0.world_off[6]);
  }
  TraceCtx cx{ctr, nullptr, nullptr};
  if constexpr (tr_mode(TR) != TR_BVH2) {
    __shared__ int s_node[kStack * kTraceBlock];
    __shared__ float s_t[kStack * kTraceBlock];
    cx.st_node = to_lds(s_node + threadIdx.x);
    cx.st_t = to_lds(s_t + threadIdx.x);
  }
  const uint64_t t_staged = tr_mode(TR) == TR_BVH4_TIMED ? __builtin_amdgcn_s_memtime() : 0;
  uint64_t t_ray = t_staged, t_hit = t_staged;
  int q = blockIdx.x * blockDim.x + threadIdx.x;
  int n = *count;
  int p = -1, fam = -1;
  if (q < n) {
    p = active[q];
    float4 ro = ntl(&P.ray_o[p]), rdv = ntl(&P.ray_d[p]);
    Ray r{v3(ro.x, ro.y, ro.z), v3(rdv.x, rdv.y, rdv.z), ro.w};
    Rng rng{ntl(&P.lcg[p]), ntl(&P.pcg[p])};
    if (tr_mode(TR) == TR_BVH4_TIMED) {
      __builtin_amdgcn_s_waitcnt(0);
      t_ray = __builtin_amdgcn_s_memtime();
    }
    WorldHit w = world_hit<MEDIA, TR>(S, r, rng, cx);
    if (tr_mode(TR) == TR_BVH4_TIMED) t_hit = __builtin_amdgcn_s_memtime();
    if (MEDIA) nts(&P.lcg[p], rng.lcg);
    store_hit(S, P, p, w, max_depth, fam);
  }
  append4(fam, p, lists, list_cap, fam_count);
  if (tr_mode(TR) == TR_BVH4_TIMED && ctr && n >= (1 << 20) && __lane_id() == 0) {
    const unsigned long long k = atomicAdd(ctr, 1ull);
    if (k < kTimingCap) {
      unsigned long long* e = ctr + 1 + 8 * k;
      e[0] = __builtin_amdgcn_s_memtime() - t_start;
      e[1] = cx.mesh_cycles;
      e[2] = (unsigned long long)cx.mesh_steps;
      e[3] = t_staged - t_start;
      e[4] = t_ray - t_staged;
      e[5] = t_hit - t_ray;
      e[6] = __builtin_amdgcn_s_memtime() - t_hit;
    }
  }
}

__global__ void __launch_bounds__(256) k_record(SceneView S, PathState P, const int* active, const int* count) {
  const int n = *count;
  for (int q = blockIdx.x * blockDim.x + threadIdx.x; q < n; q += gridDim.x * blockDim.x) {
    const int p = active[q];
    const int4 hw = ntl(&P.hit_w[p]);
    if (hw.x < 0 || hw.w < 0) continue;
    const float4 ro = ntl(&P.ray_o[p]), rdv = ntl(&P.ray_d[p]);
    const Ray r{v3(ro.x, ro.y, ro.z), v3(rdv.x, rdv.y, rdv.z), ro.w};
    const HitRec h = world_record(S, r, WorldHit{hw.x, hw.y, __int_as_float(hw.z)});
    nts(&P.hit_p[p], make_float4(h.p.x, h.p.y, h.p.z, h.u));
    nts(&P.hit_n[p], make_float4(h.n.x, h.n.y, h.n.z, h.v));
  }
}

template <bool MEDIA, int TR, int MODE>
__global__ void __launch_bounds__(kTraceBlock) k_probe(SceneView S, PathState P, const int* active, const int* count,
                                                       int* sink) {
  TraceCtx cx{nullptr, nullptr, nullptr};
  if constexpr (TR != TR_BVH2) {
    __shared__ int s_node[kStack * kTraceBlock];
    __shared__ float s_t[kStack * kTraceBlock];
    cx.st_node = to_lds(s_node + threadIdx.x);
    cx.st_t = to_lds(s_t + threadIdx.x);
  }
  int q = blockIdx.x * blockDim.x + threadIdx.x;
  if (q >= *count) return;
  int p = active[q];
  float4 ro = ntl(&P.ray_o[p]), rdv = ntl(&P.ray_d[p]);
  Ray r{v3(ro.x, ro.y, ro.z), v3(rdv.x, rdv.y, rdv.z), ro.w};
  float acc = ro.x + rdv.y;
  if (MODE >= 1) {
    Rng rng{ntl(&P.lcg[p]), ntl(&P.pcg[p])};
    WorldHit w{-1, -1, 0};
    if (MODE == 1 || MODE == 4 || MODE == 5) {
      float closest = FLT_MAX;
      for (int k = 0; k < S.n_world; ++k) {
        const DObj ob = wload<TR>(S.objs, k);
        if (ob.kind == OBJ_MEDIUM) continue;
        if (ob.kind == OBJ_MESH) {
          if (MODE == 1) continue;
          const Ray lr = chain_in(S, ob, r);
          const DMesh m = wload<TR>(S.meshes, ob.idx);
          const V3 inv = v3(1.0f / lr.d.x, 1.0f / lr.d.y, 1.0f / lr.d.z);
          const float len = length(lr.d);
          const V3 dir = lr.d / len;
          acc += inv.x + inv.y + inv.z + dir.x + dir.y + dir.z + (float)m.node4_off;
          if (MODE == 5) {
            const float4* N = S.node4 + 8 * (size_t)m.node4_off;
            float4 a = N[0], b = N[3], c = N[6];
            acc += (a.x - lr.o.x) * inv.x + (b.y - lr.o.y) * inv.y + c.z;
          }
          continue;
        }
        ObjHit h;
        if (basic_hit<TR>(S, ob, chain_in(S, ob, r), 0.001f, closest, false, h, cx)) { closest = h.t; w.obj = k; }
      }
      acc += closest;
    } else {
      w = world_hit<MEDIA, TR>(S, r, rng, cx);
      acc += w.t;
      if (MODE == 3 && w.obj >= 0) {
        HitRec h = world_record(S, r, w);
        acc += h.p.x + h.n.y + h.u;
      }
    }
    acc += (float)w.obj;
  }
  if (acc == 1234.5678f) sink[0] = p;
}

__device__ void finish_path(const PathState& P, int p, V3 C, int depth, uint64_t spec, int max_depth) {
  for (int k = depth - 1; k >= 0; --k) {
    float4 a = ntl(&P.rec_a[(size_t)p * max_depth + k]);
    V3 av = v3(a.x, a.y, a.z);
    if ((spec >> k) & 1) C = av * C;
    else C = v3(0.f) + (av * C) / a.w;
  }
  if (P.raw) {
    P.raw[3 * (size_t)p] = C.x;
    P.raw[3 * (size_t)p + 1] = C.y;
    P.raw[3 * (size_t)p + 2] = C.z;
  }
  if (!(C.x == C.x)) C.x = 0;
  if (!(C.y == C.y)) C.y = 0;
  if (!(C.z == C.z)) C.z = 0;
  nts(&P.sample[3 * (size_t)p], C.x);
  nts(&P.sample[3 * (size_t)p + 1], C.y);
  nts(&P.sample[3 * (size_t)p + 2], C.z);
}

SRR_D V3 hit_emitted(const SceneView& S, int mat, V3 rdir, V3 hpt, V3 nrm, float hu, float hv) {
  if (mat < 0) return v3(0.f);
  const DMat& M = S.mats[mat];
  if (M.kind == MAT_DIFFUSE_LIGHT && dot(nrm, rdir) < 0.0) return tex_value(S, M.tex, hu, hv, hpt);
  return v3(0.f);
}

constexpr uint32_t kSpecMark = 0x7f800001u;

template <int F>
SRR_D void scatter(const SceneView& S, const DMat& M, V3 rdir, float rtime, V3 hpt, V3 nrm, float hu, float hv,
                   Rng& rng, float4& rec, bool& spec, V3& ndir, float& ntime, int* attempts = nullptr) {
  ntime = 0.0f;
  if (F == FAM_SPEC) {
    V3 atten;
    if (M.kind == MAT_METAL) {
      V3 ud = unit_vector(rdir);
      V3 refl = ud - 2 * dot(ud, nrm) * nrm;
      ndir = refl + M.p[3] * random_in_unit_sphere(rng);
      atten = v3(M.p[0], M.p[1], M.p[2]);
    } else if (M.kind == MAT_DIELECTRIC) {
      float ri = M.p[0];
      atten = v3(1.0f, 1.0f, 1.0f);
      V3 reflected = rdir - 2 * dot(rdir, nrm) * nrm;
      V3 outward;
      float ni_over_nt, cosine;
      if (dot(rdir, nrm) > 0) {
        outward = -nrm;
        ni_over_nt = ri;
        cosine = dot(rdir, nrm) / length(rdir);
      } else {
        outward = nrm;
        ni_over_nt = 1.0 / ri;
        cosine = -dot(rdir, nrm) / length(rdir);
      }
      V3 uv = unit_vector(rdir);
      float dt = dot(uv, outward);
      float disc = 1.0 - ni_over_nt * ni_over_nt * (1 - dt * dt);
      float reflect_prob;
      V3 refracted;
      if (disc > 0) {
        refracted = ni_over_nt * (uv - outward * dt) - outward * rsqrt_exact(disc);
        float r0 = (1 - ri) / (1 + ri);
        r0 = r0 * r0;
        reflect_prob = r0 + (1 - r0) * ::pow((double)(1 - cosine), 5.0);
      } else {
        reflect_prob = 1.0;
      }
      float r01 = drand(rng);
      ndir = (r01 < reflect_prob) ? reflected : refracted;
    } else {
      ndir = random_in_unit_sphere(rng);
      atten = tex_value(S, M.tex, hu, hv, hpt);
    }
    rec = make_float4(atten.x, atten.y, atten.z, __uint_as_float(kSpecMark));
    spec = true;
  } else {
    V3 atten = tex_value(S, M.tex, hu, hv, hpt);
    Bsdf f;
    f.kind = (F == FAM_BECK) ? (int)MAT_BECKMANN : M.kind;
    f.n = nrm;
    f.uvw = onb_from_w(nrm);
    f.A = M.p[0];
    f.B = M.p[1];
    f.dist.ax = M.p[0];
    f.dist.ay = M.p[1];
    f.beck_pdf = 0;
    bsdf_prepare<F == FAM_BECK>(f, rdir);
    float pdf_val = 0;
    if (S.n_lights > 0) {
      (void)drand(rng);
      for (int guard = 0; pdf_val == 0 && guard < kMixtureGuard; ++guard) {
        if (attempts) ++*attempts;
        if (drand(rng) < 0.5) ndir = lights_random(S, hpt, rng);
        else ndir = bsdf_generate<F == FAM_BECK>(f, rdir, rng);
        pdf_val = 0.5 * lights_pdf(S, hpt, ndir) + 0.5 * bsdf_value<F == FAM_BECK>(f, rdir, ndir);
      }
    } else {
      ndir = bsdf_generate<F == FAM_BECK>(f, rdir, rng);
      pdf_val = bsdf_value<F == FAM_BECK>(f, rdir, ndir);
    }
    float spdf = scattering_pdf<F == FAM_BECK>(f, nrm, rdir, ndir);
    V3 as = atten * spdf;
    rec = make_float4(as.x, as.y, as.z, pdf_val);
    spec = false;
    ntime = rtime;
  }
}

template <int F>
SRR_D bool shade_one(const SceneView& S, const PathState& P, int p, int max_depth) {
  float4 ro = ntl(&P.ray_o[p]), rdv = ntl(&P.ray_d[p]);
  V3 rdir = v3(rdv.x, rdv.y, rdv.z);
  int depth = ntl(&P.depth[p]);
  uint64_t spec = ntl(&P.spec[p]);
  if (P.rays) P.rays[p] += 1;
  const int mat = ntl(&P.hit_w[p]).w;
  if (F == FAM_TERM) {
    V3 emitted = v3(0.f);
    if (mat >= 0) {
      float4 hp = ntl(&P.hit_p[p]), hn = ntl(&P.hit_n[p]);
      emitted = hit_emitted(S, mat, rdir, v3(hp.x, hp.y, hp.z), v3(hn.x, hn.y, hn.z), hp.w, hn.w);
    }
    finish_path(P, p, emitted, depth, spec, max_depth);
    return false;
  }
  float4 hp = ntl(&P.hit_p[p]), hn = ntl(&P.hit_n[p]);
  V3 hpt = v3(hp.x, hp.y, hp.z), nrm = v3(hn.x, hn.y, hn.z);
  const DMat M = S.mats[mat];
  Rng rng{ntl(&P.lcg[p]), ntl(&P.pcg[p])};
  V3 ndir;
  float ntime;
  float4 rec;
  bool sp;
  scatter<F>(S, M, rdir, ro.w, hpt, nrm, hp.w, hn.w, rng, rec, sp, ndir, ntime);
  nts(&P.rec_a[(size_t)p * max_depth + depth], rec);
  if (sp) spec |= (1ull << depth);
  nts(&P.ray_o[p], make_float4(hpt.x, hpt.y, hpt.z, ntime));
  nts(&P.ray_d[p], make_float4(ndir.x, ndir.y, ndir.z, 0.f));
  nts(&P.lcg[p], rng.lcg);
  nts(&P.pcg[p], rng.pcg);
  nts(&P.depth[p], depth + 1);
  nts(&P.spec[p], spec);
  return true;
}

#ifndef SRR_REC_NT
#define SRR_REC_NT 0
#endif
#ifndef SRR_FOLD4
#define SRR_FOLD4 1
#endif
SRR_D void rec_store(float4* p, float4 v) {
  if (SRR_REC_NT) nts(p, v);
  else *p = v;
}
SRR_D float4 rec_load(const float4* p) { return SRR_REC_NT ? ntl(p) : *p; }

constexpr int kPathsBlock = 256;
constexpr unsigned long long kPoolChunk = 64;

#ifndef SRR_RAYRING
#define SRR_RAYRING 1
#endif
#ifndef SRR_DIAG_VARIANTS
#define SRR_DIAG_VARIANTS 0
#endif
constexpr int kRingWords = 11;

constexpr int kPathsLdsNodesBig =
    (160 * 1024 - 8192 - 8 * kPathsLdsStack * 1024 - 1024 - (SRR_RAYRING ? 4 * kRingWords * 1024 : 0)) / 128;
constexpr int kPathsLdsNodesSmall = SRR_RAYRING ? 8 : kPathsLdsNodes;

SRR_D void path_camera_ray(const SceneView& S, const PathWork& W, uint32_t idx, Ray& r, Rng& rng) {
  const uint32_t lp = udiv31(idx, W.div_spp), s = idx - lp * (uint32_t)W.spp_w;
  if ((int)lp >= W.npix || (int)s >= W.spp_w) atomicOr(W.err, 1);
  const int pix = W.pixels ? W.pixels[lp] : lp;
  V3 o, d;
  float tm;
  double sx, sy;
  sobol2_point((uint32_t)(W.s_base + (int)s), sx, sy);
  camera_ray(S, pix, W.s_base + s, sx, sy, W.nx, W.ny, W.base_seed, o, d, tm, rng, &W.div_nx);
  r = Ray{o, d, tm};
}

template <int BS>
SRR_D void ring_put(lds_ptr<float> e, const Ray& r, const Rng& rng) {
  e[0] = r.o.x;
  e[BS] = r.o.y;
  e[2 * BS] = r.o.z;
  e[3 * BS] = r.d.x;
  e[4 * BS] = r.d.y;
  e[5 * BS] = r.d.z;
  e[6 * BS] = r.tm;
  e[7 * BS] = __uint_as_float((uint32_t)rng.lcg);
  e[8 * BS] = __uint_as_float((uint32_t)(rng.lcg >> 32));
  e[9 * BS] = __uint_as_float((uint32_t)rng.pcg);
  e[10 * BS] = __uint_as_float((uint32_t)(rng.pcg >> 32));
}

template <int BS>
SRR_D void ring_get(lds_ptr<const float> e, Ray& r, Rng& rng) {
  r = Ray{v3(e[0], e[BS], e[2 * BS]), v3(e[3 * BS], e[4 * BS], e[5 * BS]), e[6 * BS]};
  rng.lcg = (uint64_t)__float_as_uint(e[7 * BS]) | ((uint64_t)__float_as_uint(e[8 * BS]) << 32);
  rng.pcg = (uint64_t)__float_as_uint(e[9 * BS]) | ((uint64_t)__float_as_uint(e[10 * BS]) << 32);
}

struct PathsArgs {
  SceneView S;
  PathWork W;
};
#if defined(__HIP_DEVICE_COMPILE__)
template <class T>
using kptr = const __attribute__((address_space(4))) T*;
SRR_D kptr<PathsArgs> paths_args() {
  kptr<PathsArgs> p = (kptr<PathsArgs>)__builtin_amdgcn_kernarg_segment_ptr();
  asm volatile("" : "+s"(p));
  return p;
}
#else
SRR_D const PathsArgs* paths_args() { return nullptr; }
#endif

template <bool MEDIA, bool ALLFAM, int MINB, bool TIMED = false, bool WL = true, bool QUAD = false, bool CQ = false,
          int BS = kPathsBlock, bool SP = false>
#ifdef SRR_NUM_VGPR
#define SRR_PATHS_VGPR_ATTR __attribute__((amdgpu_num_vgpr(SRR_NUM_VGPR)))
#else
#define SRR_PATHS_VGPR_ATTR
#endif
__global__ void __launch_bounds__(BS, MINB) SRR_PATHS_VGPR_ATTR k_paths(PathsArgs A) {
  static_assert(BS == kPathsBlock || BS == 1024, "block size");
  (void)A;
  uint64_t tp[8] = {0, 0, 0, 0, 0, 0, 0, 0};
  uint64_t tf[20] = {0, 0, 0, 0, 0, 0, 0, 0, 0, 0, 0, 0, 0, 0, 0, 0, 0, 0, 0, 0};
  uint64_t it = 0;
  constexpr int TR = TR_BVH4_PRUNE | (WL ? TR_WL : 0) | (QUAD ? TR_QUAD : 0) | (CQ ? TR_Q : 0) | (BS == 1024 ? TR_BIG : 0) |
                     ((SP && !QUAD && !CQ) ? TR_SUSP : 0);
  __shared__ uint4 s_world[WL ? kWorldLdsBytes / 16 : 1];
  const auto view = [&]() {
    SceneView S = paths_args()->S;
    if constexpr (WL) {
      const char* b = (const char*)s_world;
      S.objs = (const DObj*)(b + S.world_off[0]);
      S.xforms = (const DXform*)(b + S.world_off[1]);
      S.spheres = (const DSphere*)(b + S.world_off[2]);
      S.rects = (const DRect*)(b + S.world_off[3]);
      S.stris = (const DStandaloneTri*)(b + S.world_off[4]);
      S.meshes = (const DMesh*)(b + S.world_off[5]);
      S.media = (const DMedium*)(b + S.world_off[6]);
      S.mats = (const DMat*)(b + S.world_off[7]);
      S.texs = (const DTex*)(b + S.world_off[8]);
      S.lights = (const DLight*)(b + S.world_off[9]);
    }
    return S;
  };
  const auto work = []() { return PathWork(paths_args()->W); };
  __shared__ int s_node[kStack * BS];
  __shared__ float s_t[kStack * BS];
  constexpr bool RING = SRR_RAYRING && !QUAD;
  constexpr int kNodesLds = BS == 1024 ? kPathsLdsNodesBig : ((WL && RING) ? kPathsLdsNodesSmall : kPathsLdsNodes);
  __shared__ float4 s_n4[kNodesLds * 8];
  __shared__ float s_ring[RING ? kRingWords * BS : 1];
  const lds_ptr<float> ringw = to_lds(s_ring + (RING ? (threadIdx.x & ~63u) : 0));
  uint32_t ring_base = 0;
  const uint32_t n_paths = (uint32_t)paths_args()->W.n_paths;
  const uint64_t t_start = paths_args()->W.wave_times ? __builtin_amdgcn_s_memrealtime() : 0;
  {
    const SceneView S0 = paths_args()->S;
    if constexpr (WL)
      for (int i = threadIdx.x; i < S0.world_words; i += blockDim.x) s_world[i] = S0.world_blob[i];
    const int n_lds_nodes = CQ ? min(S0.node4_total, 2 * kNodesLds) : min(S0.node4_total, kNodesLds);
    if (CQ)
      for (int i = threadIdx.x; i < n_lds_nodes * 4; i += blockDim.x) s_n4[i] = S0.node4q[i];
    else
      for (int i = threadIdx.x; i < n_lds_nodes * 8; i += blockDim.x) s_n4[i] = S0.node4[i];
  }
  __syncthreads();
  const int slot = blockIdx.x * blockDim.x + threadIdx.x;
  const auto rec_at = [&](const PathWork& W, int k) -> float4* {
    int s = slot;
    asm volatile("" : "+v"(s));
    return W.rec + ((size_t)k * W.lanes + s);
  };
  int g = -1;
  uint32_t pool = 0, pool_end = 0;
  uint32_t nxt_lane0 = 0;
  bool nxt_armed = false;
  uint32_t nxt_base = 0;
  bool nxt_ready = false;
  Ray r{};
  Rng rng{};
  int depth = 0;
  int walking = 0;
  uint32_t nrays = 0;
  uint32_t n_events = 0;
  constexpr uint32_t kCapped = 1, kSuspended = 1u << 12;
  uint32_t n_iter = 0, max_rounds = 0;
  for (;;) {
    ++n_iter;
    uint64_t tq = TIMED ? __builtin_amdgcn_s_memtime() : 0;
    const bool need = g < 0;
    const uint64_t nm = __ballot(need);
    if (nm && pool < n_paths) {
      const SceneView S = view();
      const PathWork W = work();
      const uint32_t cnt = __popcll(nm);
      const uint32_t rank = __popcll(nm & ((1ull << lane_id()) - 1));
      const uint32_t avail = pool_end - pool;
      uint32_t idx = 0;
      if (RING) {
        if (need && rank < avail) {
          const uint32_t i0 = pool + rank;
          if (i0 < n_paths) {
            g = (int)i0;
            ring_get<BS>(ringw + (i0 - ring_base), r, rng);
            depth = 0;
          }
        }
        if (avail >= cnt) {
          pool += cnt;
        } else {
          uint32_t nb;
          if (nxt_armed) {
            nb = nxt_ready ? nxt_base : __builtin_amdgcn_readfirstlane(nxt_lane0);
            nxt_armed = false;
            nxt_ready = false;
          } else {
            uint32_t b = 0;
            if (lane_id() == 0) b = (uint32_t)atomicAdd(W.cursor, (unsigned long long)kPoolChunk);
            nb = __builtin_amdgcn_readfirstlane(b);
          }
          const uint32_t gi = nb + (uint32_t)lane_id();
          if (gi < n_paths) {
            Ray gr;
            Rng grng;
            path_camera_ray(S, W, gi, gr, grng);
            ring_put<BS>(ringw + lane_id(), gr, grng);
          }
          __builtin_amdgcn_fence(__ATOMIC_SEQ_CST, "wavefront");
          ring_base = nb;
          if (need && rank >= avail) {
            const uint32_t i1 = nb + (rank - avail);
            if (i1 < n_paths) {
              g = (int)i1;
              ring_get<BS>(ringw + (i1 - nb), r, rng);
              depth = 0;
            }
          }
          pool = nb + (cnt - avail);
          pool_end = nb + (uint32_t)kPoolChunk;
        }
      } else if (avail >= cnt) {
        idx = pool + rank;
        pool += cnt;
      } else {
        uint32_t nb;
        if (nxt_armed) {
          nb = nxt_ready ? nxt_base : __builtin_amdgcn_readfirstlane(nxt_lane0);
          nxt_armed = false;
          nxt_ready = false;
        } else {
          uint32_t b = 0;
          if (lane_id() == 0) b = (uint32_t)atomicAdd(W.cursor, (unsigned long long)kPoolChunk);
          nb = __builtin_amdgcn_readfirstlane(b);
        }
        idx = rank < avail ? pool + rank : nb + (rank - avail);
        pool = nb + (cnt - avail);
        pool_end = nb + (uint32_t)kPoolChunk;
      }
      if (!RING && need && idx < n_paths) {
        g = (int)idx;
        path_camera_ray(S, W, idx, r, rng);
        depth = 0;
      }
    }
    if (!nxt_armed && pool_end < n_paths) {
      if (lane_id() == 0) nxt_lane0 = (uint32_t)atomicAdd(paths_args()->W.cursor, (unsigned long long)kPoolChunk);
      nxt_armed = true;
    }
    if (__ballot(g >= 0) == 0) break;
    if (TIMED) tf[9] += __popcll(__ballot(g >= 0));
    if (TIMED) {
      __builtin_amdgcn_s_waitcnt(0);
      const uint64_t t = __builtin_amdgcn_s_memtime();
      tp[0] += t - tq;
      tq = t;
      ++it;
    }
    bool done = false;
    V3 C = v3(0.f);
    bool diff = false, pend = false;
    int natt = 0;
    uint64_t fam_dt[3] = {0, 0, 0};
    DiffSetup ds{};
    V3 d_atten = v3(0.f), d_n = v3(0.f), d_dir = v3(0.f);
    float d_pdf = 0;
    int d_tries = 0;
    bool d_dead = false;
    WorldHit w{-1, -1, 0};
    if (g >= 0) {
      const SceneView S = view();
      const PathWork W = work();
      TraceCtx cx{nullptr, to_lds(s_node + threadIdx.x), to_lds(s_t + threadIdx.x)};
      cx.lds_nodes = (const __attribute__((address_space(3))) f32x4*)to_lds(s_n4);
      cx.lds_count = CQ ? min(S.node4_total, 2 * kNodesLds) : min(S.node4_total, kNodesLds);
      cx.st_cap = min(W.stack_cap, kStack);
      cx.ovf = W.counters + 11;
      cx.gst = W.gstack;
      cx.gst_cap = W.gstack ? W.gstack_cap : 0;
      cx.gst_stride = W.lanes;
      cx.slot = slot;
      if constexpr ((TR & TR_SUSP) != 0) {
        cx.walk_thr = vreg((int)((__popcll(__ballot(true)) * (uint32_t)paths_args()->W.walk_q) >> 6));
        cx.resume = walking;
        cx.susp = vreg(0);
      }
#ifdef SRR_SLOW_RAYS
      const uint64_t t_w0 = __builtin_amdgcn_s_memrealtime();
      cx.last_steps = 0;
      const Ray r_in = r;
#endif
      w = world_hit<MEDIA, TIMED ? (TR_BVH4_TIMED | (WL ? TR_WL : 0) | (SP ? TR_SUSP : 0)) : TR>(S, r, rng, cx);
      if constexpr ((TR & TR_SUSP) != 0) {
        walking = cx.susp;
        if (walking) {
          w.obj = -1;
          n_events += kSuspended;
        }
      }
#ifdef SRR_SLOW_RAYS
      const uint64_t t_w = __builtin_amdgcn_s_memrealtime() - t_w0;
      if ((t_w > (uint64_t)SRR_SLOW_RAYS || (cx.last_steps & (1 << 28))) && W.slow_rays) {
        const unsigned q = atomicAdd(W.slow_count, 1u);
        if (q < 65536u) {
          float* e = W.slow_rays + 16 * (size_t)q;
          e[0] = __int_as_float(g);
          e[1] = __int_as_float(depth);
          e[2] = r_in.o.x; e[3] = r_in.o.y; e[4] = r_in.o.z;
          e[5] = r_in.d.x; e[6] = r_in.d.y; e[7] = r_in.d.z;
          e[8] = r_in.tm;
          e[9] = __int_as_float((int)t_w);
          e[10] = __int_as_float(cx.last_steps);
          e[11] = __int_as_float(w.obj);
          e[12] = __int_as_float(w.prim);
          e[13] = w.t;
          e[14] = __int_as_float(slot);
          e[15] = __int_as_float((int)(t_w0 & 0x7fffffff));
        }
      }
#endif
      if (TIMED) {
        const uint64_t t = __builtin_amdgcn_s_memtime();
        tp[1] += t - tq - cx.mesh_cycles;
        tp[2] += cx.mesh_cycles;
        tf[10] += cx.mesh_steps;
        tf[11] += cx.mesh_lane_steps;
        tf[12] += cx.mesh_walkers;
        tf[13] += cx.leaf_cycles;
        tf[14] += cx.leaf_passes;
        tf[15] += cx.step_parts[0];
        tf[16] += cx.step_parts[1];
        tf[17] += cx.step_parts[2];
        tq = t;
      }
      done = !walking;
    }
    if (nxt_armed && !nxt_ready) {
      nxt_base = __builtin_amdgcn_readfirstlane(nxt_lane0);
      nxt_ready = true;
    }
    if (g >= 0) {
      if (w.obj >= 0) {
        const SceneView S = view();
        const PathWork W = work();
        const HitRec h = world_record<TR>(S, r, w);
        const int kind = h.mat >= 0 ? S.mats[h.mat].kind : -1;
        if (TIMED) {
          __builtin_amdgcn_s_waitcnt(0);
          const uint64_t t = __builtin_amdgcn_s_memtime();
          tp[5] += t - tq;
          tq = t;
        }
        const int fam = family_of(h.mat, kind, depth, W.max_depth);
        if (TIMED) {
          const uint64_t mb = __ballot(fam == FAM_BECK), ms = __ballot(fam == FAM_SPEC),
                         md = __ballot(fam == FAM_DIFF && S.n_lights > 0);
          tf[3] += mb != 0; tf[4] += ms != 0; tf[5] += md != 0;
          tf[6] += __popcll(mb); tf[7] += __popcll(ms); tf[8] += __popcll(md);
        }
        if (fam == FAM_TERM) {
          C = hit_emitted(S, h.mat, r.d, h.p, h.n, h.u, h.v);
        } else if ((!ALLFAM || fam == FAM_DIFF) && S.n_lights > 0) {
          const DMat M = S.mats[h.mat];
          d_atten = tex_value(S, M.tex, h.u, h.v, h.p);
          Bsdf f;
          f.kind = M.kind;
          f.n = h.n;
          f.uvw = onb_from_w(h.n);
          f.A = M.p[0];
          f.B = M.p[1];
          bsdf_prepare<false>(f, r.d);
          ds = diff_setup(f, h.p);
          if (SRR_MIXTURE_SKIP) d_dead = bsdf_dead(S, f, h.p);
          (void)drand(rng);
          d_n = h.n;
          diff = pend = true;
          done = false;
          if (TIMED) fam_dt[2] = __builtin_amdgcn_s_memtime() - tq;
        } else {
          const DMat M = S.mats[h.mat];
          float4 rec;
          bool sp;
          V3 nd;
          float nt;
          const uint64_t tb = TIMED ? __builtin_amdgcn_s_memtime() : 0;
          if (!ALLFAM || fam == FAM_DIFF) scatter<FAM_DIFF>(S, M, r.d, r.tm, h.p, h.n, h.u, h.v, rng, rec, sp, nd, nt);
          else if (fam == FAM_BECK) {
            scatter<FAM_BECK>(S, M, r.d, r.tm, h.p, h.n, h.u, h.v, rng, rec, sp, nd, nt, TIMED ? &natt : nullptr);
            if (TIMED) fam_dt[0] = __builtin_amdgcn_s_memtime() - tb;
          } else {
            scatter<FAM_SPEC>(S, M, r.d, r.tm, h.p, h.n, h.u, h.v, rng, rec, sp, nd, nt);
            if (TIMED) fam_dt[1] = __builtin_amdgcn_s_memtime() - tb;
          }
          if (depth >= W.max_depth || slot >= W.lanes) atomicOr(W.err, 2);
          else rec_store(rec_at(W, depth), rec);
          if (!sp && S.n_lights > 0 && rec.w == 0) n_events += kCapped;
          r = Ray{h.p, nd, nt};
          ++depth;
          done = false;
        }
      }
    }
    if (TIMED) {
      int sum = natt, mx = natt;
      for (int o = 32; o > 0; o >>= 1) {
        sum += __shfl_xor(sum, o);
        mx = max(mx, __shfl_xor(mx, o));
      }
      tf[18] += sum;
      tf[19] += mx;
      for (int q = 0; q < 3; ++q) {
        uint64_t m = fam_dt[q];
        for (int o = 32; o > 0; o >>= 1) m = max(m, (uint64_t)__shfl_xor((unsigned long long)m, o));
        tf[q] += m;
      }
    }
    if (__ballot(pend)) {
      const SceneView S = view();
      const uint64_t tc = TIMED ? __builtin_amdgcn_s_memtime() : 0;
      int rounds = 0;
      if (SRR_MIXTURE_SKIP == 1) {
        rounds = skip_mixture(S, ds, d_dead, pend, d_tries, rng.lcg, d_dir, d_pdf);
      } else {
        if (SRR_MIXTURE_SKIP == 2) rounds = skip_mixture(S, ds, d_dead, pend, d_tries, rng.lcg, d_dir, d_pdf, 1);
        if (__ballot(pend)) rounds += coop_mixture(S, ds, pend, d_tries, rng.lcg, d_dir, d_pdf, paths_args()->W.deep_tries);
      }
      if (TIMED) {
        tp[6] += __builtin_amdgcn_s_memtime() - tc;
        tp[7] += rounds;
      }
      max_rounds = max(max_rounds, (uint32_t)rounds);
    }
    if (diff) {
      const PathWork W = work();
      if (d_pdf == 0) n_events += kCapped;
      float c = dot(d_n, unit_vector(d_dir));
      if (c < 0) c = 0;
      const V3 as = d_atten * (c / kPi);
      if (depth >= W.max_depth || slot >= W.lanes) atomicOr(W.err, 2);
      else rec_store(rec_at(W, depth), make_float4(as.x, as.y, as.z, d_pdf));
      r = Ray{ds.p, d_dir, r.tm};
      ++depth;
    }
    if (g >= 0) {
      const PathWork W = work();
      if (TIMED) {
        const uint64_t t = __builtin_amdgcn_s_memtime();
        tp[3] += t - tq;
        tq = t;
      }
      if (done && (g >= W.n_paths || depth > W.max_depth)) {
        atomicOr(W.err, 4);
        g = -1;
        done = false;
      }
      if (done) {
#if SRR_FOLD4
        int k = depth - 1;
        for (; k >= 0; k -= 4) {
          float4 a[4];
#pragma unroll
          for (int j = 0; j < 4; ++j) a[j] = k - j >= 0 ? rec_load(rec_at(W, k - j)) : make_float4(0, 0, 0, 0);
#pragma unroll
          for (int j = 0; j < 4; ++j) {
            if (k - j < 0) break;
            const V3 av = v3(a[j].x, a[j].y, a[j].z);
            if (__float_as_uint(a[j].w) == kSpecMark) C = av * C;
            else C = v3(0.f) + (av * C) / a[j].w;
          }
        }
#else
        for (int k = depth - 1; k >= 0; --k) {
          const float4 a = rec_load(rec_at(W, k));
          const V3 av = v3(a.x, a.y, a.z);
          if (__float_as_uint(a.w) == kSpecMark) C = av * C;
          else C = v3(0.f) + (av * C) / a.w;
        }
#endif
        if (W.raw) {
          const size_t kq = (size_t)(g / W.spp_w) * W.keep_spp + W.keep_s0 + (size_t)(g % W.spp_w);
          W.raw[3 * kq] = C.x;
          W.raw[3 * kq + 1] = C.y;
          W.raw[3 * kq + 2] = C.z;
          W.rays[kq] = (uint8_t)(depth + 1);
        }
        if (!(C.x == C.x)) C.x = 0;
        if (!(C.y == C.y)) C.y = 0;
        if (!(C.z == C.z)) C.z = 0;
        nts(&W.sample[3 * (size_t)g], C.x);
        nts(&W.sample[3 * (size_t)g + 1], C.y);
        nts(&W.sample[3 * (size_t)g + 2], C.z);
        nrays += depth + 1;
        g = -1;
      }
      if (TIMED) tp[4] += __builtin_amdgcn_s_memtime() - tq;
    }
  }
  const PathWork W = work();
  if (TIMED && lane_id() == 0) {
    for (int q = 0; q < 5; ++q) atomicAdd(W.counters + 4 + q, (unsigned long long)tp[q]);
    atomicAdd(W.counters + 9, (unsigned long long)it);
    atomicAdd(W.counters + 10, (unsigned long long)tp[5]);
    atomicAdd(W.counters + 13, (unsigned long long)tp[6]);
    atomicAdd(W.counters + 14, (unsigned long long)tp[7]);
    for (int q = 0; q < 20; ++q) atomicAdd(W.counters + 16 + q, (unsigned long long)tf[q]);
  }

  unsigned long long tot = nrays;
  for (int o = 32; o > 0; o >>= 1) tot += __shfl_xor(tot, o);
  if (lane_id() == 0 && tot) atomicAdd(W.counters, tot);
  if (__ballot(n_events != 0)) {
    unsigned long long cap = n_events & (kSuspended - 1), su = n_events / kSuspended;
    for (int o = 32; o > 0; o >>= 1) {
      cap += __shfl_xor(cap, o);
      su += __shfl_xor(su, o);
    }
    if (lane_id() == 0) {
      if (cap) atomicAdd(W.counters + 15, cap);
      if (su) atomicAdd(W.counters + 36, su);
    }
  }
  if (W.wave_times && lane_id() == 0) {
    const size_t wv = (size_t)(blockIdx.x * blockDim.x + threadIdx.x) / 64;
    W.wave_times[4 * wv] = t_start;
    W.wave_times[4 * wv + 1] = __builtin_amdgcn_s_memrealtime();
    W.wave_times[4 * wv + 2] = tot;
    W.wave_times[4 * wv + 3] = n_iter | ((unsigned long long)max_rounds << 32);
  }
}

constexpr int kAccChunk = 16;
struct AccOut {
  float* out;
  int scale_ns;
};
SRR_D void acc_write(float* acc, AccOut o, size_t a, float cx, float cy, float cz) {
  acc[a] = cx;
  acc[a + 1] = cy;
  acc[a + 2] = cz;
  if (o.out) {
    if (o.scale_ns) {
      const float k = 1.0 / (float)o.scale_ns;
      o.out[a] = cx * k;
      o.out[a + 1] = cy * k;
      o.out[a + 2] = cz * k;
    } else {
      o.out[a] = cx;
      o.out[a + 1] = cy;
      o.out[a + 2] = cz;
    }
  }
}

__global__ void __launch_bounds__(256) k_accumulate_window(const float* sample, int npix, int spp_w, float* acc,
                                                           int init, AccOut o) {
  __shared__ float tile[256 * (3 * kAccChunk + 1)];
  const int p0 = blockIdx.x * 256;
  const int lp = p0 + threadIdx.x;
  const int np = min(256, npix - p0);
  float cx = 0, cy = 0, cz = 0;
  if (lp < npix && !init) {
    cx = acc[3 * (size_t)lp];
    cy = acc[3 * (size_t)lp + 1];
    cz = acc[3 * (size_t)lp + 2];
  }
  for (int s0 = 0; s0 < spp_w; s0 += kAccChunk) {
    const int n = min(kAccChunk, spp_w - s0), row = 3 * n;
    for (int i = threadIdx.x; i < np * row; i += 256) {
      const int px = i / row, f = i - px * row;
      tile[px * (3 * kAccChunk + 1) + f] = ntl(&sample[((size_t)(p0 + px) * spp_w + s0) * 3 + f]);
    }
    __syncthreads();
    if (lp < npix) {
      const float* t = &tile[threadIdx.x * (3 * kAccChunk + 1)];
      for (int k = 0; k < n; ++k) {
        cx += t[3 * k];
        cy += t[3 * k + 1];
        cz += t[3 * k + 2];
      }
// ... 25 lines not shown
#pragma unroll
      for (int j = 0; j < kQ; ++j) {
        const int i = threadIdx.x + 256 * j, px = i / kQ, f4 = i - px * kQ;
        v[j] = ntl(&base[((size_t)px * spp_w + s0) * 3 / 4 + f4]);
      }
    };
    if (s_full > 0) fetch(0);
    for (int s0 = 0; s0 < s_full; s0 += kAccChunk) {
#pragma unroll
      for (int j = 0; j < kQ; ++j) {
        const int i = threadIdx.x + 256 * j, px = i / kQ, f4 = i - px * kQ;
        float* d = &tile[px * (3 * kAccChunk + 1) + 4 * f4];
        d[0] = v[j].x;
        d[1] = v[j].y;
        d[2] = v[j].z;
        d[3] = v[j].w;
      }
      __syncthreads();
      if (s0 + kAccChunk < s_full) fetch(s0 + kAccChunk);
      const float* t = &tile[threadIdx.x * (3 * kAccChunk + 1)];
#pragma unroll
      for (int k = 0; k < kAccChunk; ++k) {
        cx += t[3 * k];
        cy += t[3 * k + 1];
        cz += t[3 * k + 2];
      }
      __syncthreads();
    }
  } else {
    for (int s0 = 0; s0 < s_full; s0 += kAccChunk) {
      for (int i = threadIdx.x; i < np * kQ; i += 256) {
        const int px = i / kQ, f4 = i - px * kQ;
        const float4 v = ntl(&sample4[((size_t)(p0 + px) * spp_w + s0) * 3 / 4 + f4]);
        float* d = &tile[px * (3 * kAccChunk + 1) + 4 * f4];
        d[0] = v.x;
        d[1] = v.y;
        d[2] = v.z;
        d[3] = v.w;
      }
      __syncthreads();
      if (lp < npix) {
        const float* t = &tile[threadIdx.x * (3 * kAccChunk + 1)];
#pragma unroll
        for (int k = 0; k < kAccChunk; ++k) {
          cx += t[3 * k];
          cy += t[3 * k + 1];
          cz += t[3 * k + 2];
        }
      }
      __syncthreads();
    }
  }
  if (s_full < spp_w) {
    const int n = spp_w - s_full, qn = 3 * n / 4;
    for (int i = threadIdx.x; i < np * qn; i += 256) {
      const int px = i / qn, f4 = i - px * qn;
      const float4 v = ntl(&sample4[((size_t)(p0 + px) * spp_w + s_full) * 3 / 4 + f4]);
      float* d = &tile[px * (3 * kAccChunk + 1) + 4 * f4];
      d[0] = v.x;
      d[1] = v.y;
      d[2] = v.z;
      d[3] = v.w;
    }
    __syncthreads();
    if (lp < npix) {
      const float* t = &tile[threadIdx.x * (3 * kAccChunk + 1)];
      for (int k = 0; k < n; ++k) {
        cx += t[3 * k];
        cy += t[3 * k + 1];
        cz += t[3 * k + 2];
      }
    }
  }
  if (lp >= npix) return;
  acc_write(acc, o, 3 * (size_t)lp, cx, cy, cz);
}

constexpr int kMaxRegions = 8;

template <int F>
__global__ void __launch_bounds__(256) k_shade(SceneView S, PathState P, const int* lists, int list_cap,
                                               const int* fam_count, int* next, int* next_count, int* region_alive,
                                               int region_size, int max_depth) {
  __shared__ int hist[kMaxRegions];
  if (threadIdx.x < kMaxRegions) hist[threadIdx.x] = 0;
  __syncthreads();
  const int* list = lists + (size_t)F * list_cap;
  const int n = fam_count[F];
  for (int base = blockIdx.x * blockDim.x; base < n; base += gridDim.x * blockDim.x) {
    int q = base + threadIdx.x;
    bool alive = false;
    int p = -1;
    if (q < n) {
      p = list[q];
      alive = shade_one<F>(S, P, p, max_depth);
    }
    if (F != FAM_TERM) {
      append(alive, p, next, next_count);
      if (alive) atomicAdd(&hist[p / region_size], 1);
    }
  }
  if (F != FAM_TERM) {
    __syncthreads();
    if (threadIdx.x < kMaxRegions && hist[threadIdx.x]) atomicAdd(&region_alive[threadIdx.x], hist[threadIdx.x]);
  }
}

__global__ void __launch_bounds__(256) k_accumulate(PathState P, BatchInfo B, float* acc) {
  int lp = blockIdx.x * blockDim.x + threadIdx.x;
  if (lp >= B.n_paths / B.spp_batch) return;
  size_t a = 3 * (size_t)(B.p0 + lp);
  float cx = acc[a], cy = acc[a + 1], cz = acc[a + 2];
  for (int s = 0; s < B.spp_batch; ++s) {
    size_t q = 3 * ((size_t)B.slot0 + (size_t)lp * B.spp_batch + s);
    cx += ntl(&P.sample[q]);
    cy += ntl(&P.sample[q + 1]);
    cz += ntl(&P.sample[q + 2]);
  }
  acc[a] = cx;
  acc[a + 1] = cy;
  acc[a + 2] = cz;
}

__global__ void k_finish(const float* acc, float* mean, int64_t n, int ns) {
  int64_t i = (int64_t)blockIdx.x * blockDim.x + threadIdx.x;
  if (i >= 3 * n) return;
  float k = 1.0 / (float)ns;
  mean[i] = acc[i] * k;
}

__global__ void k_scatter_pixels(const float* __restrict__ packed, const int32_t* __restrict__ index, int64_t n,
                                 float* __restrict__ image) {
  const int64_t i = (int64_t)blockIdx.x * blockDim.x + threadIdx.x;
  if (i >= 3 * n) return;
  const int64_t px = i / 3;
  image[3 * (int64_t)index[px] + (i - 3 * px)] = packed[i];
}

__global__ void __launch_bounds__(256) k_merl_lookup(const double* table, int64_t n, const double* angles,
                                                     double* rgb, int32_t* cell) {
  const int64_t q = (int64_t)blockIdx.x * blockDim.x + threadIdx.x;
  if (q >= n) return;
  const double* a = angles + 4 * q;
  const int c = merl::cell_of(a[0], a[1], a[2], a[3]);
  double r, g, b;
  merl::rgb_of(table, c, r, g, b);
  rgb[3 * q] = r;
  rgb[3 * q + 1] = g;
  rgb[3 * q + 2] = b;
  if (cell) cell[q] = c;
}

enum KatKind : int { KAT_ERF, KAT_BECK11, KAT_BECK_DIST, KAT_BECK_PDF, KAT_COSINE, KAT_ORENNAYAR, KAT_DIELECTRIC,
                     KAT_METAL, KAT_TRIANGLE, KAT_AABB, KAT_SQRT, KAT_CAMERA, KAT_LIGHTS, KAT_LIGHT_LIST };

SRR_D V3 kat3(const float* p) { return v3(p[0], p[1], p[2]); }
SRR_D void kat_put3(float* p, V3 v) { p[0] = v.x, p[1] = v.y, p[2] = v.z; }
SRR_D uint64_t kat_lcg(const float* p) { return (uint64_t)p[0] | ((uint64_t)p[1] << 24); }
SRR_D void kat_put_lcg(float* p, uint64_t s) { p[0] = (float)(s & 0xFFFFFF), p[1] = (float)((s >> 24) & 0xFFFFFF); }
SRR_D uint64_t kat_pcg(const float* p) {
  uint64_t s = 0;
  for (int k = 0; k < 4; ++k) s |= (uint64_t)p[k] << (16 * k);
  return s;
}
SRR_D void kat_put_pcg(float* p, uint64_t s) {
  for (int k = 0; k < 4; ++k) p[k] = (float)((s >> (16 * k)) & 0xFFFF);
}

__global__ void k_kat(int kind, int n, int w, float* rec, const float* aux, const DStandaloneTri* tris, KatTables kt) {
  const int q = blockIdx.x * blockDim.x + threadIdx.x;
  if (q >= n) return;
  float* r = rec + (size_t)q * w;
  const float* a = aux + 4 * (size_t)q;
  switch (kind) {
    case KAT_ERF:
      r[1] = Erf(r[0]);
      r[2] = ErfInv(r[0]);
      break;
    case KAT_BECK11:
      beckmann_sample11(r[0], r[1], r[2], r[3], r[4]);
      break;
    case KAT_BECK_DIST: {
      const Beck d{a[0], a[1]};
      const V3 wo = kat3(r + 2);
      const V3 wh = beckmann_sample_wh(d, wo, r[5], r[6]);
      r[7] = d.ax;
      r[8] = d.ay;
      kat_put3(r + 9, wh);
      r[12] = d.D(wh);
      r[13] = d.G(wo, wh);
      r[14] = d.Pdf(wo, wh);
      r[15] = d.Lambda(wo);
      break;
    }
    case KAT_BECK_PDF: {
      Bsdf f;
      f.kind = MAT_BECKMANN;
      f.n = kat3(r + 2);
      f.uvw = onb_from_w(f.n);
      f.dist = Beck{a[0], a[1]};
      f.beck_pdf = 0;
      const V3 wo = kat3(r + 5);
      Rng rng{0, kat_pcg(r + 8)};
      bsdf_prepare<true>(f, wo);
      const V3 wi = bsdf_generate<true>(f, wo, rng);
      kat_put3(r + 12, wi);
      r[15] = bsdf_value<true>(f, wo, wi);
      r[16] = scattering_pdf<true>(f, f.n, wo, wi);
      kat_put_pcg(r + 17, rng.pcg);
      break;
    }
    case KAT_COSINE:
    case KAT_ORENNAYAR: {
      Bsdf f;
      f.kind = kind == KAT_COSINE ? MAT_LAMBERTIAN : MAT_ORENNAYAR;
      f.n = kat3(r + 1);
      f.uvw = onb_from_w(f.n);
      f.A = a[0];
      f.B = a[1];
      const V3 wo = kat3(r + 4);
      bsdf_prepare<false>(f, wo);
      Rng rng{kat_lcg(r + 7), 0};
      const V3 d = bsdf_generate<false>(f, wo, rng);
      r[9] = a[0];
      r[10] = a[1];
      kat_put3(r + 11, d);
      r[14] = bsdf_value<false>(f, wo, d);
      r[15] = bsdf_value<false>(f, wo, kat3(r + 16));
      kat_put_lcg(r + 19, rng.lcg);
      break;
    }
    case KAT_DIELECTRIC:
    case KAT_METAL: {
      DMat M{};
      if (kind == KAT_DIELECTRIC) {
        M.kind = MAT_DIELECTRIC;
        M.p[0] = r[0];
      } else {
        M.kind = MAT_METAL;
        M.p[0] = M.p[1] = M.p[2] = 0.5f;
        M.p[3] = r[0] < 1 ? r[0] : 1;
      }
      Rng rng{kat_lcg(r + 7), 0};
      float4 rc;
      bool sp;
      V3 nd;
      float nt;
      scatter<FAM_SPEC>(SceneView{}, M, kat3(r + 1), 0.25f, v3(1, 2, 3), kat3(r + 4), 0, 0, rng, rc, sp, nd, nt);
      kat_put3(r + 9, nd);
      kat_put_lcg(r + 12, rng.lcg);
      break;
    }
    case KAT_TRIANGLE: {
      SceneView S{};
      S.stris = tris;
      const DObj ob{OBJ_TRI, 0, 0, q};
      const Ray ray{kat3(r + 9), kat3(r + 12), 0.0f};
      float t = 0;
      const bool h = prim_hit<TR_WL>(S, ob, ray, 0.001f, FLT_MAX, r[15] != 0, t);
      HitRec hr;
      hr.u = hr.v = 0;
      hr.p = hr.n = v3(0.f);
      if (h) prim_record(S, ob, ray, t, -1, hr);
      r[16] = h ? 1.f : 0.f;
      r[17] = h ? t : 0;
      r[18] = hr.u;
      r[19] = hr.v;
      kat_put3(r + 20, hr.n);
      kat_put3(r + 23, hr.p);
      break;
    }
    case KAT_SQRT:
      r[1] = rsqrt_exact(r[0]);
      break;
    case KAT_CAMERA: {
      Rng rng{kat_lcg(r + 12), 0};
      V3 o, d;
      float tm;
      camera_get_ray(kt.cams[q], r[10], r[11], rng, o, d, tm);
      kat_put3(r + 14, o);
      kat_put3(r + 17, d);
      r[20] = tm;
      kat_put_lcg(r + 21, rng.lcg);
      break;
    }
    case KAT_LIGHTS:
    case KAT_LIGHT_LIST: {
      SceneView S{};
      S.rects = kt.rects;
      S.spheres = kt.spheres;
      S.stris = kt.stris;
      S.lights = kt.lights;
      S.n_lights = kt.n_lights;
      S.light_weight = kt.n_lights > 0 ? (float)(1.0 / kt.n_lights) : 0.f;
      Rng rng{kat_lcg(r + 3), 0};
      const V3 o = kat3(r);
      V3 d1, d2;
      float p1, p2;
      if (kind == KAT_LIGHTS) {
        d1 = light_random_one(S, kt.lights[0], o, rng);
        p1 = light_pdf_one(S, kt.lights[0], o, d1);
        d2 = light_random_one(S, kt.lights[1], o, rng);
        p2 = light_pdf_one(S, kt.lights[1], o, d2);
      } else {
        d1 = lights_random(S, o, rng);
        p1 = lights_pdf(S, o, d1);
        d2 = light_random_one(S, kt.lights[2], o, rng);
        p2 = light_pdf_one(S, kt.lights[2], o, d2);
      }
      kat_put3(r + 5, d1);
      r[8] = p1;
      kat_put3(r + 9, d2);
      r[12] = p2;
      kat_put_lcg(r + 13, rng.lcg);
      break;
    }
    case KAT_AABB: {
      const V3 d = kat3(r + 9);
      r[14] = slab(make_float4(r[0], r[1], r[2], 0), make_float4(r[3], r[4], r[5], 0), kat3(r + 6),
                   v3(1.0f / d.x, 1.0f / d.y, 1.0f / d.z), r[12], r[13]) ? 1.f : 0.f;
      break;
    }
  }
}

}

void launch_raygen(const SceneView& S, const PathState& P, const BatchInfo& B, hipStream_t st) {
  int g = (B.n_paths + 255) / 256;
  hipLaunchKernelGGL(dev::k_raygen, dim3(g), dim3(256), 0, st, S, P, B);
}
static unsigned long long* g_timing = nullptr;

void dump_trace_timing() {
  if (!g_timing) return;
  std::vector<unsigned long long> v(1 + 8 * dev::kTimingCap);
  (void)hipDeviceSynchronize();
  (void)hipMemcpy(v.data(), g_timing, v.size() * sizeof(unsigned long long), hipMemcpyDeviceToHost);
  size_t n = std::min<unsigned long long>(v[0], dev::kTimingCap);
  std::vector<double> tot, mesh, steps, per, stg, ray, hit, tail;
  for (size_t k = 0; k < n; ++k) {
    const unsigned long long* e = &v[1 + 8 * k];
    stg.push_back((double)e[3]);
    ray.push_back((double)e[4]);
    hit.push_back((double)e[5]);
    tail.push_back((double)e[6]);
    tot.push_back((double)e[0]);
    mesh.push_back((double)e[1]);
    steps.push_back((double)e[2]);
    if (e[2] > 0) per.push_back((double)e[1] / (double)e[2]);
  }
  auto pct = [](std::vector<double> x, double q) {
    if (x.empty()) return 0.0;
    std::sort(x.begin(), x.end());
    return x[std::min(x.size() - 1, (size_t)(q * x.size()))];
  };
  auto mean = [](const std::vector<double>& x) {
    double a = 0;
    for (double y : x) a += y;
    return x.empty() ? 0.0 : a / x.size();
  };
  fprintf(stderr, "trace timing: %zu waves (s_memtime ticks)\n", n);
  for (auto [name, x] : {std::pair<const char*, std::vector<double>*>{"wave total", &tot}, {"mesh", &mesh},
                         {"mesh steps (wave max)", &steps}, {"ticks per step", &per}, {"LDS staging", &stg},
                         {"ray load", &ray}, {"world hit", &hit}, {"store+append", &tail}})
    fprintf(stderr, "  %-22s mean %10.1f  p10 %10.1f  p50 %10.1f  p90 %10.1f  p99 %10.1f\n", name, mean(*x), pct(*x, .1),
            pct(*x, .5), pct(*x, .9), pct(*x, .99));
}

void launch_trace(const SceneView& S, const PathState& P, const int* active, const int* count, int max_n,
                  int* lists, int list_cap, int* fam_count, int* fetch, int max_depth, unsigned long long* ctr,
                  hipStream_t st) {
  int g = (max_n + 255) / 256;
  static const int tr = [] {
    const char* e = getenv("SRR_TRAVERSAL");
    if (e && !strcmp(e, "bvh2")) return (int)dev::TR_BVH2;
    if (e && !strcmp(e, "bvh4")) return (int)dev::TR_BVH4;
    if (e && !strcmp(e, "bvh4prune")) return (int)dev::TR_BVH4_PRUNE;
    if (e && !strcmp(e, "timed")) return (int)dev::TR_BVH4_TIMED;
    return (int)dev::TR_BVH4_PRUNE;
  }();
  const int grec = std::min(g, 2048);
  static unsigned long long* timing = nullptr;
  if (tr == dev::TR_BVH4_TIMED && !timing) {
    (void)hipMalloc((void**)&timing, (1 + 8 * dev::kTimingCap) * sizeof(unsigned long long));
    (void)hipMemset(timing, 0, (1 + 8 * dev::kTimingCap) * sizeof(unsigned long long));
    g_timing = timing;
  }
  unsigned long long* kctr = tr == dev::TR_BVH4_TIMED ? timing : ctr;
#define SRR_LAUNCH_TRACE(M, T)                                                                        \
  hipLaunchKernelGGL((dev::k_trace<M, T>), dim3(g), dim3(dev::kTraceBlock), 0, st, S, P, active, count, \
                     lists, list_cap, fam_count, max_depth, kctr)
  const bool wl = S.world_words * 16 <= dev::kWorldLdsBytes && !getenv("SRR_NO_WORLD_LDS");
#define SRR_LAUNCH_TRACE_W(M, T)                  \
  if (wl) SRR_LAUNCH_TRACE(M, (T) | dev::TR_WL); \
  else SRR_LAUNCH_TRACE(M, T);
#define SRR_LAUNCH_TRACE_M(M)                                                 \
  if (trm == dev::TR_BVH2) { SRR_LAUNCH_TRACE_W(M, dev::TR_BVH2) }            \
  else if (trm == dev::TR_BVH4) { SRR_LAUNCH_TRACE_W(M, dev::TR_BVH4) }       \
  else if (trm == dev::TR_BVH4_TIMED) { SRR_LAUNCH_TRACE_W(M, dev::TR_BVH4_TIMED) } \
  else { SRR_LAUNCH_TRACE_W(M, dev::TR_BVH4_PRUNE) }
  const int trm = tr;
  if (S.has_media) {
    SRR_LAUNCH_TRACE_M(true)
  } else {
    SRR_LAUNCH_TRACE_M(false)
  }
  hipLaunchKernelGGL(dev::k_record, dim3(grec), dim3(256), 0, st, S, P, active, count);
  static const bool probe = getenv("SRR_PROBE") && getenv("SRR_PROBE")[0] == '1';
  if (probe && !S.has_media) {
    static int* sink = nullptr;
    if (!sink) (void)hipMalloc((void**)&sink, 16);
#define SRR_PROBE(T, M) \
  hipLaunchKernelGGL((dev::k_probe<false, T, M>), dim3(g), dim3(dev::kTraceBlock), 0, st, S, P, active, count, sink)
#define SRR_PROBES(T) SRR_PROBE(T, 0); SRR_PROBE(T, 1); SRR_PROBE(T, 4); SRR_PROBE(T, 5); SRR_PROBE(T, 2);
    if (trm == dev::TR_BVH2) { SRR_PROBES(dev::TR_BVH2) }
    else if (trm == dev::TR_BVH4) { SRR_PROBES(dev::TR_BVH4) }
    else { SRR_PROBES(dev::TR_BVH4_PRUNE) }
#undef SRR_PROBES
#undef SRR_PROBE
  }
#undef SRR_LAUNCH_TRACE_M
#undef SRR_LAUNCH_TRACE_W
#undef SRR_LAUNCH_TRACE
}
void launch_shade(const SceneView& S, const PathState& P, const int* lists, int list_cap, const int* fam_count,
                  int* next, int* next_count, int* region_alive, int region_size, int max_n, int max_depth,
                  hipStream_t st) {
  int g = std::min((max_n + 255) / 256, 2048);
  hipLaunchKernelGGL(dev::k_shade<dev::FAM_DIFF>, dim3(g), dim3(256), 0, st, S, P, lists, list_cap, fam_count, next,
                     next_count, region_alive, region_size, max_depth);
  hipLaunchKernelGGL(dev::k_shade<dev::FAM_BECK>, dim3(g), dim3(256), 0, st, S, P, lists, list_cap, fam_count, next,
                     next_count, region_alive, region_size, max_depth);
  hipLaunchKernelGGL(dev::k_shade<dev::FAM_SPEC>, dim3(g), dim3(256), 0, st, S, P, lists, list_cap, fam_count, next,
                     next_count, region_alive, region_size, max_depth);
  hipLaunchKernelGGL(dev::k_shade<dev::FAM_TERM>, dim3(g), dim3(256), 0, st, S, P, lists, list_cap, fam_count, next,
                     next_count, region_alive, region_size, max_depth);
}
void launch_accumulate(const PathState& P, const BatchInfo& B, float* acc, hipStream_t st) {
  int np = B.n_paths / B.spp_batch;
  int g = (np + 255) / 256;
  hipLaunchKernelGGL(dev::k_accumulate, dim3(g), dim3(256), 0, st, P, B, acc);
}
void launch_finish(const float* acc, float* mean, int64_t n, int ns, hipStream_t st) {
  int64_t g = (3 * n + 255) / 256;
  hipLaunchKernelGGL(dev::k_finish, dim3((unsigned)g), dim3(256), 0, st, acc, mean, n, ns);
}

void launch_scatter_pixels(const float* packed, const int32_t* index, int64_t n, float* image, hipStream_t st) {
  if (n <= 0) return;
  const int64_t g = (3 * n + 255) / 256;
  hipLaunchKernelGGL(dev::k_scatter_pixels, dim3((unsigned)g), dim3(256), 0, st, packed, index, n, image);
}


constexpr int kPathsOccDefault = 4;
static int paths_min_blocks() {
  static const int v = [] {
    const char* e = getenv("SRR_PATHS_OCC");
    int x = e ? atoi(e) : kPathsOccDefault;
    return x >= 2 && x <= 6 ? x : kPathsOccDefault;
  }();
  return v;
}

int paths_block_lanes(const SceneView& S) {
  static const bool big = [] {
    const char* e = getenv("SRR_BIGBLOCK");
    return !e || atoi(e) != 0;
// ... 113 lines not shown
```

### simple-raytracing-render_amd/csrc/renderer.cpp

```cpp
#include "renderer.h"

#include "multi.h"

#include <algorithm>
#include <chrono>
#include <cstdlib>
#include <cstring>
#include <memory>
#include <thread>
#include <cstdio>

namespace srr {

constexpr int kCtrWords = 40;
constexpr int kVisitWords = 3 + 2 * 64;

#define RCHK(x)                                                        \
  do {                                                                 \
    hipError_t e_ = (x);                                               \
    if (e_ != hipSuccess) {                                            \
      err = std::string(#x) + ": " + hipGetErrorString(e_);            \
      return SRR_EIO;                                                  \
    }                                                                  \
  } while (0)

template <class T>
static hipError_t upload(T** dst, const std::vector<T>& v, std::vector<void*>& keep) {
  size_t bytes = std::max<size_t>(v.size() * sizeof(T), 16);
  hipError_t e = hipMalloc((void**)dst, bytes);
  if (e != hipSuccess) return e;
  keep.push_back(*dst);
  if (!v.empty()) e = hipMemcpy(*dst, v.data(), v.size() * sizeof(T), hipMemcpyHostToDevice);
  return e;
}

int renderer_create(const Scene& sc, int device, srr_renderer** out, std::string& err) {
  Flat F;
  int rc = flatten(sc, F, err);
  if (rc < 0) return rc;
  return renderer_create_flat(F, device, out, err);
}

int renderer_create_flat(const Flat& F, int device, srr_renderer** out, std::string& err) {
  std::unique_ptr<srr_renderer> r(new srr_renderer());
  r->device = device;
  if (const char* e = getenv("SRR_LANES")) r->n_lanes = std::max(1, std::min(kMaxLanes, atoi(e)));
  RCHK(hipSetDevice(device));
  std::vector<void*>& K = r->scene_bufs;
  DObj* objs; DXform* xf; DSphere* sph; DRect* rct; DStandaloneTri* st; DMesh* me; float* nodes; float* n4;
  float* tp; TriShade* ts; DMedium* md; DMat* mt; DTex* tx; uint8_t* im; float* pr; int32_t* pp; DLight* li;
  DCamera* cm;
  DObvh* ob;
  DObvhChild* oc;
  DSGroup* sg;
  DSGItem* sgi;
  std::vector<DCamera> cam{F.cam};
  RCHK(upload(&objs, F.objs, K));
  RCHK(upload(&xf, F.xforms, K));
  RCHK(upload(&sph, F.spheres, K));
  RCHK(upload(&rct, F.rects, K));
  RCHK(upload(&st, F.stris, K));
  RCHK(upload(&me, F.meshes, K));
  RCHK(upload(&nodes, F.nodes, K));
  RCHK(upload(&n4, F.node4, K));
  float* n4q;
  RCHK(upload(&n4q, F.node4q, K));
  RCHK(upload(&tp, F.tri_pos, K));
  float* tedge;
  {
    const size_t nt = F.tri_pos.size() / 16;
    std::vector<float> pr(32 * nt, 0.f);
    for (size_t i = 0; i < nt; ++i)
      for (int j = 0; j < 2; ++j) {
        const float* q = &F.tri_pos[16 * std::min(i + j, nt - 1)];
        float* o = &pr[32 * i + 9 * j];
        for (int c = 0; c < 3; ++c) {
          o[c] = q[c];
          o[3 + c] = q[4 + c] - q[c];
          o[6 + c] = q[8 + c] - q[c];
        }
      }
    RCHK(upload(&tedge, pr, K));
  }
  RCHK(upload(&ts, F.tri_shade, K));
  RCHK(upload(&md, F.media, K));
  RCHK(upload(&ob, F.obvhs, K));
  RCHK(upload(&oc, F.obvh_children, K));
  RCHK(upload(&sg, F.sgroups, K));
  RCHK(upload(&sgi, F.sg_items, K));
  RCHK(upload(&mt, F.mats, K));
  RCHK(upload(&tx, F.texs, K));
  RCHK(upload(&im, F.images, K));
  RCHK(upload(&pr, F.perlin_ranvec, K));
  RCHK(upload(&pp, F.perlin_perm, K));
  RCHK(upload(&li, F.lights, K));
  RCHK(upload(&cm, cam, K));
  std::vector<uint8_t> blob;
  int off[10];
  auto put = [&](int k, const void* data, size_t bytes) {
    off[k] = (int)blob.size();
    blob.insert(blob.end(), (const uint8_t*)data, (const uint8_t*)data + bytes);
    blob.resize((blob.size() + 15) & ~(size_t)15, 0);
  };
  put(0, F.objs.data(), F.objs.size() * sizeof(DObj));
  put(1, F.xforms.data(), F.xforms.size() * sizeof(DXform));
  put(2, F.spheres.data(), F.spheres.size() * sizeof(DSphere));
  put(3, F.rects.data(), F.rects.size() * sizeof(DRect));
  put(4, F.stris.data(), F.stris.size() * sizeof(DStandaloneTri));
  put(5, F.meshes.data(), F.meshes.size() * sizeof(DMesh));
  put(6, F.media.data(), F.media.size() * sizeof(DMedium));
  put(7, F.mats.data(), F.mats.size() * sizeof(DMat));
  put(8, F.texs.data(), F.texs.size() * sizeof(DTex));
  put(9, F.lights.data(), F.lights.size() * sizeof(DLight));
  uint8_t* wb;
  RCHK(upload(&wb, blob, K));
  SceneView& V = r->view;
  V.world_blob = (const uint4*)wb;
  V.world_words = (int)(blob.size() / 16);
  for (int k = 0; k < 10; ++k) V.world_off[k] = off[k];
  V.objs = objs;
  V.n_world = F.n_world;
  V.has_media = F.media.empty() ? 0 : 1;
  V.xforms = xf;
  V.spheres = sph;
  V.rects = rct;
  V.stris = st;
  V.meshes = me;
  V.nodes = (const float4*)nodes;
  V.node4 = (const float4*)n4;
  V.node4_lds = (int)std::min<size_t>(kPathsLdsNodes, F.node4.size() / 32);
  V.node4_total = (int)(F.node4.size() / 32);
  V.node4q = F.node4q_ok && !F.node4q.empty() ? (const float4*)n4q : nullptr;
  V.node4_lds_q = (int)std::min<size_t>(2 * kPathsLdsNodes, F.node4q.size() / kNode4qWords);
  {
    const char* e = getenv("SRR_CBVH");
    V.use_q = V.node4q && e && atoi(e) != 0;
  }
  {
    const char* e = getenv("SRR_QUAD");
    V.quad_trace = e ? (atoi(e) != 0) : false;
    const char* q = getenv("SRR_QUAD_MAX");
    V.quad_max = q ? atoi(q) : 32;
  }
  {
    int n_mesh = 0;
    V.mesh_obj = -1;
    for (int k = 0; k < F.n_world; ++k)
      if (F.objs[k].kind == OBJ_MESH) {
        ++n_mesh;
        V.mesh_obj = k;
      }
    if (n_mesh != 1) V.mesh_obj = -1;
  }
  V.tri_pos = (const float4*)tp;
  V.tri_edge = (const float4*)tedge;
  V.tri_shade = ts;
  V.media = md;
  V.obvhs = ob;
  V.obvh_children = oc;
  V.sgroups = sg;
  V.sg_items = sgi;
  V.mats = mt;
  V.texs = tx;
  V.images = im;
  V.perlin_ranvec = pr;
  V.perlin_perm = pp;
  V.lights = li;
  V.n_lights = (int)F.lights.size();
  V.light_weight = V.n_lights > 0 ? (float)(1.0 / V.n_lights) : 0.f;
  V.cam = cm;
  r->has_meshes = !F.meshes.empty() || !F.obvhs.empty();
  r->diffuse_only = true;
  for (const DMat& m : F.mats)
    if (m.kind != MAT_LAMBERTIAN && m.kind != MAT_ORENNAYAR && m.kind != MAT_DIFFUSE_LIGHT) r->diffuse_only = false;
  {
    int max_tris = 0;
    for (const DMesh& m : F.meshes) max_tris = std::max(max_tris, (int)m.n_tris);
    r->walk_q_default = (!F.meshes.empty() && (!r->diffuse_only || V.has_media || max_tris >= 20000)) ? 8 : 0;
  }
  RCHK(hipStreamCreateWithFlags(&r->acc_st, hipStreamNonBlocking));
  RCHK(hipEventCreate(&r->ev_beg));
  RCHK(hipEventCreate(&r->ev_end));
  RCHK(hipEventCreateWithFlags(&r->ev_async_in, hipEventDisableTiming));
  for (int l = 0; l < kMaxLanes; ++l) {
    Lane& L = r->lanes[l];
    RCHK(hipStreamCreateWithFlags(&L.st, hipStreamNonBlocking));
    RCHK(hipEventCreate(&L.ev_t0));
    RCHK(hipEventCreate(&L.ev_t1));
    RCHK(hipEventCreate(&L.ev_s1));
    RCHK(hipEventCreateWithFlags(&L.ev_rb, hipEventDisableTiming));
    for (int k = 0; k < kRegionsPerLane; ++k) {
      RCHK(hipEventCreateWithFlags(&L.done_ev[k], hipEventDisableTiming));
      RCHK(hipEventCreateWithFlags(&L.acc_ev[k], hipEventDisableTiming));
    }
    RCHK(hipMalloc((void**)&L.cnt, 16 * sizeof(int32_t)));
    RCHK(hipHostMalloc((void**)&L.rb, 16 * sizeof(int32_t)));
  }
  *out = r.release();
  return 0;
}

static void free_lane_paths(Lane& L) {
  for (void* p : L.bufs) (void)hipFree(p);
  L.bufs.clear();
  L.cap = 0;
  L.P = PathState{};
  L.act[0] = L.act[1] = nullptr;
  L.lists = nullptr;
}

template <class T>
static hipError_t lane_alloc(Lane& L, T** p, size_t n) {
  hipError_t e = hipMalloc((void**)p, std::max<size_t>(n * sizeof(T), 16));
  if (e == hipSuccess) L.bufs.push_back(*p);
  return e;
}

static int ensure_lane(Lane& L, size_t n, int depth, bool keep, std::string& err) {
  int d = std::max(depth, 1);
  if (n <= L.cap && d <= L.cap_depth && (!keep || L.has_raw)) return 0;
  free_lane_paths(L);
  PathState& P = L.P;
  RCHK(lane_alloc(L, &P.ray_o, n));
  RCHK(lane_alloc(L, &P.ray_d, n));
  RCHK(lane_alloc(L, &P.lcg, n));
  RCHK(lane_alloc(L, &P.pcg, n));
  RCHK(lane_alloc(L, &P.depth, n));
  RCHK(lane_alloc(L, &P.spec, n));
  RCHK(lane_alloc(L, &P.hit_w, n));
  RCHK(lane_alloc(L, &P.hit_p, n));
  RCHK(lane_alloc(L, &P.hit_n, n));
  RCHK(lane_alloc(L, &P.rec_a, n * d));
  RCHK(lane_alloc(L, &P.sample, 3 * n));
  RCHK(lane_alloc(L, &L.lists, 4 * n));
  RCHK(lane_alloc(L, &L.act[0], n));
  RCHK(lane_alloc(L, &L.act[1], n));
  L.has_raw = keep;
  if (keep) {
    RCHK(lane_alloc(L, &P.raw, 3 * n));
    RCHK(lane_alloc(L, &P.rays, n));
  }
  L.cap = n;
  L.cap_depth = d;
  return 0;
}

static void accum_key(const srr_params* p, int key[5]) {
  const bool whole = p->shard_count <= 1;
  key[0] = p->nx;
  key[1] = p->ny;
  key[2] = whole ? 0 : p->shard_index;
  key[3] = whole ? 1 : p->shard_count;
  key[4] = whole ? 0 : p->tile;
}

static int begin_accum(srr_renderer* r, const srr_params* p, int64_t npix, hipStream_t st, std::string& err,
                       bool* zero_pending = nullptr) {
  if (zero_pending) *zero_pending = false;
  int key[5];
  accum_key(p, key);
  if (p->flags & SRR_FLAG_CONTINUE) {
    if (r->acc_npix != npix) {
      err = "SRR_FLAG_CONTINUE: no running sums for this shard (render without the flag or srr_accum_set first)";
      return SRR_EINVAL;
    }
    if (p->sample_begin != r->acc_samples) {
      err = "SRR_FLAG_CONTINUE: sample_begin " + std::to_string(p->sample_begin) + " != the " +
            std::to_string(r->acc_samples) + " samples already in the running sums";
      return SRR_EINVAL;
    }
    if (r->acc_key[0] >= 0 && !std::equal(key, key + 5, r->acc_key)) {
      err = "SRR_FLAG_CONTINUE: the running sums belong to another frame or shard";
      return SRR_EINVAL;
    }
    std::copy(key, key + 5, r->acc_key);
    return 0;
  }
  if (zero_pending) *zero_pending = true;
  else RCHK(hipMemsetAsync(r->acc, 0, 3 * npix * sizeof(float), st));
  r->acc_npix = npix;
  r->acc_samples = 0;
  std::copy(key, key + 5, r->acc_key);
  return 0;
}

static hipError_t stage_pixels(srr_renderer* r, const int32_t* pix, int64_t npix, bool identity) {
  r->pix_key[0] = -1;
  if ((size_t)npix > r->pix_cap) {
    (void)hipFree(r->pixels);
    (void)hipFree(r->acc);
    r->pixels = nullptr;
    r->acc = nullptr;
    r->pix_cap = 0;
    r->acc_npix = 0;
    r->acc_samples = 0;
    std::fill(r->acc_key, r->acc_key + 5, -1);
    hipError_t e = hipMalloc((void**)&r->pixels, npix * sizeof(int32_t));
    if (e == hipSuccess) e = hipMalloc((void**)&r->acc, 3 * npix * sizeof(float));
    if (e != hipSuccess) return e;
    r->pix_cap = npix;
  }
  r->pix_identity = identity;
  return identity ? hipSuccess : hipMemcpy(r->pixels, pix, npix * sizeof(int32_t), hipMemcpyHostToDevice);
}

static hipError_t ensure_sobol(srr_renderer* r, int n_sobol) {
  if (n_sobol <= r->sobol_n) return hipSuccess;
  (void)hipFree(r->sobol);
  r->sobol = nullptr;
  r->sobol_n = 0;
  hipError_t e = hipMalloc((void**)&r->sobol, 2 * (size_t)n_sobol * sizeof(double));
  if (e != hipSuccess) return e;
  std::vector<double> sp(2 * (size_t)n_sobol);
  sobol2((unsigned)n_sobol, sp.data());
  e = hipMemcpy(r->sobol, sp.data(), sp.size() * sizeof(double), hipMemcpyHostToDevice);
  if (e == hipSuccess) r->sobol_n = n_sobol;
  return e;
}

struct AccCommit {
  srr_renderer* r;
  bool ok = false;
// ... 691 lines not shown
```

Baseline: 9058.

## Pre-resolve light and material records on host and specialize single-rect-light sampling

Builds resolved light records that inline the rect geometry, precomputed area and max-abs extent. Builds resolved material records that inline constant texture colours. Adds a templated single-XZ-rect-light fast path through the mixture sampling, skip and dead-BSDF checks. The aim is to remove dependent loads of the rect and texture tables and the per-sample loop and branch over lights. In exchange the device structs are larger and the template instantiations add code size and register pressure.

Measured after the change: 9145, median of 6. Within noise of the previous version (+1.0%).

```diff
diff --git a/simple-raytracing-render_amd/csrc/capi.cpp b/simple-raytracing-render_amd/csrc/capi.cpp
--- a/simple-raytracing-render_amd/csrc/capi.cpp
+++ b/simple-raytracing-render_amd/csrc/capi.cpp
@@ -16,6 +16,7 @@
 #include "../../include/srr/merl.h"
 #include "multi.h"
 #include "renderer.h"
+#include "resolved.h"
 
 using namespace srr;
 
@@ -623,10 +624,10 @@
   if (!name || !records || n <= 0 || width <= 0) return fail(SRR_EINVAL, "bad KAT arguments");
   static const char* kNames[] = {"erf",   "beckmann11", "beckmann_dist", "beckmann_pdf", "cosine_pdf",
                                  "orennayar_pdf", "dielectric", "metal", "triangle", "aabb", "sqrt",
-                                 "camera", "lights", "light_list"};
-  static const int kWidth[] = {3, 5, 16, 21, 21, 21, 14, 14, 26, 15, 2, 23, 15, 15};
+                                 "camera", "lights", "light_list", "light_row"};
+  static const int kWidth[] = {3, 5, 16, 21, 21, 21, 14, 14, 26, 15, 2, 23, 15, 15, 9};
   int kind = -1;
-  for (int k = 0; k < 14; ++k)
+  for (int k = 0; k < 15; ++k)
     if (!strcmp(name, kNames[k])) kind = k;
   if (kind < 0) return fail(SRR_EINVAL, std::string("no device KAT named ") + name);
   if (width != kWidth[kind]) return fail(SRR_EINVAL, std::string("KAT ") + name + ": unexpected record width");
@@ -654,6 +655,13 @@
       std::memcpy(d.sh.n, t.n, 36);
       for (int k = 0; k < 3; ++k) d.sh.uv[2 * k] = t.uv[3 * k], d.sh.uv[2 * k + 1] = t.uv[3 * k + 1];
       d.sh.mat = -1;
+    } else if (kind == 14) {
+      DRect rq{};
+      rq.kax = 1, rq.a0 = 0, rq.a1 = 2, rq.mat = -1;
+      rq.lo0 = r[0], rq.hi0 = r[1], rq.lo1 = r[2], rq.hi1 = r[3], rq.k = r[4];
+      const DLightR row = resolve_light(DLight{LIGHT_XZRECT, 0}, std::vector<DRect>{rq});
+      aux[4 * (size_t)q] = row.area;
+      aux[4 * (size_t)q + 1] = row.mabs;
     }
   }
   std::vector<DCamera> cams(kind == 11 ? n : 1);
@@ -699,7 +707,7 @@
   DRect* d_rects = nullptr;
   DSphere* d_sph = nullptr;
   DStandaloneTri* d_stris = nullptr;
-  DLight* d_lights = nullptr;
+  DLightR* d_lights = nullptr;
   const size_t rb = (size_t)n * width * sizeof(float);
   int rc = 0;
   if (hipMalloc((void**)&d_rec, rb) != hipSuccess || hipMalloc((void**)&d_aux, aux.size() * 4) != hipSuccess ||
@@ -719,7 +727,8 @@
   upload(d_rects, lf.rects);
   upload(d_sph, lf.spheres);
   upload(d_stris, lf.stris);
-  upload(d_lights, lf.lights);
+  const std::vector<DLightR> lights_r = resolve_lights(lf.lights, lf.rects);
+  upload(d_lights, lights_r);
   const KatTables kt{d_cams, d_rects, d_sph, d_stris, d_lights, (int)lf.lights.size()};
   if (!rc && launch_kat(kind, n, width, d_rec, d_aux, d_tris, kt) < 0) rc = fail(SRR_EIO, "KAT kernel launch failed");
   if (!rc && (hipDeviceSynchronize() != hipSuccess || hipMemcpy(records, d_rec, rb, hipMemcpyDeviceToHost) != hipSuccess))
diff --git a/simple-raytracing-render_amd/csrc/device_scene.h b/simple-raytracing-render_amd/csrc/device_scene.h
--- a/simple-raytracing-render_amd/csrc/device_scene.h
+++ b/simple-raytracing-render_amd/csrc/device_scene.h
@@ -105,6 +105,14 @@
   float p[4];
 };
 
+struct DMatR {
+  int32_t kind;
+  int32_t tex;
+  float p[4];
+  float c[3];
+  int32_t c_const;
+};
+
 enum TexKind : int32_t { TEX_CONST = 0, TEX_IMAGE = 1, TEX_CHECKER = 2, TEX_NOISE = 3 };
 
 struct DTex {
@@ -122,6 +130,16 @@
   int32_t idx;
 };
 
+struct DLightR {
+  int32_t kind;
+  int32_t idx;
+  int32_t draws;
+  float lo0, hi0, lo1, hi1, k;
+  float area;
+  float mabs;
+  int32_t pad[2];
+};
+
 struct DCamera {
   float origin[3], llc[3], horizontal[3], vertical[3], u[3], v[3];
   float time0, time1, lens_radius;
diff --git a/simple-raytracing-render_amd/csrc/kernels.h b/simple-raytracing-render_amd/csrc/kernels.h
--- a/simple-raytracing-render_amd/csrc/kernels.h
+++ b/simple-raytracing-render_amd/csrc/kernels.h
@@ -34,14 +34,16 @@
   const DObvhChild* obvh_children;
   const DSGroup* sgroups;
   const DSGItem* sg_items;
-  const DMat* mats;
+  const DMatR* mats;
   const DTex* texs;
   const uint8_t* images;
   const float* perlin_ranvec;
   const int32_t* perlin_perm;
-  const DLight* lights;
+  const DLightR* lights;
   int n_lights;
   float light_weight;
+  int light_one;
+  int light_draws;
   const DCamera* cam;
   const uint4* world_blob;
   int world_words;
@@ -137,7 +139,7 @@
   const DRect* rects;
   const DSphere* spheres;
   const DStandaloneTri* stris;
-  const DLight* lights;
+  const DLightR* lights;
   int n_lights;
 };
 int launch_kat(int kind, int n, int w, float* d_rec, const float* d_aux, const DStandaloneTri* d_tris,
diff --git a/simple-raytracing-render_amd/csrc/kernels.hip b/simple-raytracing-render_amd/csrc/kernels.hip
--- a/simple-raytracing-render_amd/csrc/kernels.hip
+++ b/simple-raytracing-render_amd/csrc/kernels.hip
@@ -5,6 +5,7 @@
 #include <cstdint>
 #include <cstdlib>
 #include <cstring>
+#include <type_traits>
 
 #include "device_scene.h"
 #include "devmath.h"
@@ -37,8 +38,8 @@
   return false;
 }
 
-template <int KAX>
-SRR_D bool rect_hit_t(const DRect& q, const Ray& r, float tmin, float tmax, float& t) {
+template <int KAX, class Q>
+SRR_D bool rect_hit_t(const Q& q, const Ray& r, float tmin, float tmax, float& t) {
   constexpr int A0 = KAX == 0 ? 1 : 0, A1 = KAX == 2 ? 1 : 2;
   const float tt = (q.k - r.o[KAX]) / r.d[KAX];
   if (tt < tmin || tt > tmax) return false;
@@ -1647,6 +1648,11 @@
   return tex_value_slow(S, ti, u, v, p);
 }
 
+SRR_D V3 mat_color(const SceneView& S, const DMatR& M, float u, float v, V3 p) {
+  if (M.c_const) return v3(M.c[0], M.c[1], M.c[2]);
+  return tex_value(S, M.tex, u, v, p);
+}
+
 struct Onb {
   V3 u, v, w;
 };
@@ -1911,26 +1917,21 @@
 __device__ __noinline__ float light_pdf_other(const DSphere* spheres, const DStandaloneTri* stris, DLight L, V3 o,
                                               V3 v);
 
-SRR_D float light_pdf_one(const SceneView& S, const DLight& L, V3 o, V3 v) {
+SRR_D float rect_light_pdf(const DLightR& q, V3 o, V3 v) {
   Ray r{o, v, 0.0f};
-  if (L.kind == LIGHT_XZRECT) {
-    const DRect& q = S.rects[L.idx];
-    float t;
-#if SRR_RECTAX
-    if (rect_hit_t<1>(q, r, 0.001f, FLT_MAX, t)) {
-#else
-    float u, vv;
-    if (rect_hit(q, r, 0.001f, FLT_MAX, t, u, vv)) {
-#endif
-      float area = (q.hi0 - q.lo0) * (q.hi1 - q.lo1);
-      float distance_square = t * t * squared_length(v);
-      float cosine = fabsf(v.y / length(v));
-      return distance_square / (cosine * area);
-    }
-    return 0;
-  }
+  float t;
+  if (rect_hit_t<1>(q, r, 0.001f, FLT_MAX, t)) {
+    float distance_square = t * t * squared_length(v);
+    float cosine = fabsf(v.y / length(v));
+    return distance_square / (cosine * q.area);
+  }
+  return 0;
+}
+
+SRR_D float light_pdf_one(const SceneView& S, const DLightR& L, V3 o, V3 v) {
+  if (L.kind == LIGHT_XZRECT) return rect_light_pdf(L, o, v);
   if (L.kind == LIGHT_NONE) return 0.0;
-  return light_pdf_other(S.spheres, S.stris, L, o, v);
+  return light_pdf_other(S.spheres, S.stris, DLight{L.kind, L.idx}, o, v);
 }
 
 __device__ __noinline__ float light_pdf_other(const DSphere* spheres, const DStandaloneTri* stris, DLight L, V3 o,
@@ -1987,15 +1988,16 @@
 __device__ __noinline__ LightDraw light_random_other(const DSphere* spheres, const DStandaloneTri* stris, DLight L,
                                                      V3 o, uint64_t lcg);
 
-SRR_D V3 light_random_one(const SceneView& S, const DLight& L, V3 o, Rng& rng) {
-  if (L.kind == LIGHT_XZRECT) {
-    const DRect& q = S.rects[L.idx];
-    float z = q.lo1 + drand(rng) * (q.hi1 - q.lo1);
-    float x = q.lo0 + drand(rng) * (q.hi0 - q.lo0);
-    return v3(x, q.k, z) - o;
-  }
+SRR_D V3 rect_light_random(const DLightR& q, V3 o, Rng& rng) {
+  float z = q.lo1 + drand(rng) * (q.hi1 - q.lo1);
+  float x = q.lo0 + drand(rng) * (q.hi0 - q.lo0);
+  return v3(x, q.k, z) - o;
+}
+
+SRR_D V3 light_random_one(const SceneView& S, const DLightR& L, V3 o, Rng& rng) {
+  if (L.kind == LIGHT_XZRECT) return rect_light_random(L, o, rng);
   if (L.kind == LIGHT_NONE) return v3(1, 0, 0);
-  const LightDraw ld = light_random_other(S.spheres, S.stris, L, o, rng.lcg);
+  const LightDraw ld = light_random_other(S.spheres, S.stris, DLight{L.kind, L.idx}, o, rng.lcg);
   rng.lcg = ld.lcg;
   return ld.d;
 }
@@ -2193,20 +2195,45 @@
   return f;
 }
 
-SRR_D float mixture_attempt(const SceneView& S, Bsdf& f, V3 hpt, Rng& rng, V3& ndir) {
-  if (drand(rng) < 0.5) ndir = lights_random(S, hpt, rng);
-  else ndir = bsdf_generate<false>(f, v3(0.f), rng);
-  return 0.5 * lights_pdf(S, hpt, ndir) + 0.5 * bsdf_value<false>(f, v3(0.f), ndir);
+template <bool ONE>
+SRR_D float mixture_attempt(const SceneView& S, const DLightR& L0, Bsdf& f, V3 hpt, Rng& rng, V3& ndir) {
+  if (drand(rng) < 0.5) {
+    if (ONE) {
+      (void)drand(rng);
+      ndir = rect_light_random(L0, hpt, rng);
+    } else {
+      ndir = lights_random(S, hpt, rng);
+    }
+  } else {
+    ndir = bsdf_generate<false>(f, v3(0.f), rng);
+  }
+  float lp;
+  if (ONE) {
+    lp = 0;
+    lp += S.light_weight * rect_light_pdf(L0, hpt, ndir);
+  } else {
+    lp = lights_pdf(S, hpt, ndir);
+  }
+  return 0.5 * lp + 0.5 * bsdf_value<false>(f, v3(0.f), ndir);
 }
 
 SRR_D uint64_t lcg_step(uint64_t s) { return (0x5DEECE66DULL * s + 0xB16ULL) & 0xFFFFFFFFFFFFULL; }
 
+template <bool ONE>
 SRR_D uint64_t skip_attempt(const SceneView& S, uint64_t s) {
   s = lcg_step(s);
+  if (ONE) {
+    if ((s >> 47) == 0) s = lcg_step(s);
+    return lcg_step(lcg_step(s));
+  }
   if ((s >> 47) == 0) {
     s = lcg_step(s);
-    const int idx = int((double)(uint32_t)(s >> 16) / 4294967296.0 * S.n_lights);
-    if (S.lights[idx].kind != LIGHT_NONE) s = lcg_step(lcg_step(s));
+    int draws = S.light_draws;
+    if (draws < 0) {
+      const int idx = int((double)(uint32_t)(s >> 16) / 4294967296.0 * S.n_lights);
+      draws = S.lights[idx].draws;
+    }
+    if (draws != 0) s = lcg_step(lcg_step(s));
   } else {
     s = lcg_step(lcg_step(s));
   }
@@ -2222,8 +2249,9 @@
 #endif
 constexpr int kMaxHelpers = SRR_COOP_HELPERS;
 
-SRR_D int coop_mixture(const SceneView& S, const DiffSetup& me, bool& pend, int& tries, uint64_t& lcg, V3& ndir,
-                       float& pdf, int deep_tries) {
+template <bool ONE>
+SRR_D int coop_mixture(const SceneView& S, const DLightR& L0, const DiffSetup& me, bool& pend, int& tries, uint64_t& lcg,
+                       V3& ndir, float& pdf, int deep_tries) {
   int rounds = 0;
   const int lane = lane_id();
   const uint64_t lt = (1ull << lane) - 1;
@@ -2261,10 +2289,10 @@
     V3 nd = v3(0.f);
     float pv = 0;
     if (active) {
-      for (int j = 0; j < k; ++j) s = skip_attempt(S, s);
+      for (int j = 0; j < k; ++j) s = skip_attempt<ONE>(S, s);
       Rng rr{s, 0};
       Bsdf f = bsdf_of(d);
-      pv = mixture_attempt(S, f, d.p, rr, nd);
+      pv = mixture_attempt<ONE>(S, L0, f, d.p, rr, nd);
       s = rr.lcg;
     }
     const uint64_t ok = __ballot(active && (pv != 0 || t0 + k + 1 >= kMixtureGuard));
@@ -2333,6 +2361,16 @@
 
 SRR_D bool light_point_far(V3 c, V3 p, V3 w, float sgn, float m) { return sgn * dot(c - p, w) <= -m; }
 
+SRR_D bool rect_light_far(const DLightR& q, V3 p, V3 w, float sgn, float ps) {
+  if (!(q.k != p.y)) return false;
+  const float m = 1e-3f * (ps + q.mabs);
+  for (int c = 0; c < 4; ++c) {
+    const V3 v = v3((c & 1) ? q.hi0 : q.lo0, q.k, (c & 2) ? q.hi1 : q.lo1);
+    if (!light_point_far(v, p, w, sgn, m)) return false;
+  }
+  return true;
+}
+
 SRR_D bool bsdf_dead(const SceneView& S, const Bsdf& f, V3 p) {
   if (f.kind == MAT_LAMBERTIAN) {
     if (f.flip ? !(f.co <= 0) : !(f.co >= 0)) return false;
@@ -2342,28 +2380,11 @@
   const float sgn = f.flip ? -1.f : 1.f;
   const V3 w = f.uvw.w;
   const float ps = fmaxf(fmaxf(fabsf(p.x), fabsf(p.y)), fabsf(p.z)) + 1.f;
+  if (S.light_one) return rect_light_far(uni(S.lights[0]), p, w, sgn, ps);
   for (int k = 0; k < S.n_lights; ++k) {
-    const DLight L = S.lights[k];
+    const DLightR L = S.lights[k];
     if (L.kind == LIGHT_XZRECT) {
-      const DRect q = S.rects[L.idx];
-#if SRR_XFAX
-      if (!(q.k != p.y)) return false;
-#else
-      if (!(q.k != p[q.kax])) return false;
-#endif
-      const float m = 1e-3f * (ps + fmaxf(fmaxf(fmaxf(fabsf(q.lo0), fabsf(q.hi0)), fmaxf(fabsf(q.lo1), fabsf(q.hi1))),
-                                          fabsf(q.k)));
-      for (int c = 0; c < 4; ++c) {
-#if SRR_XFAX
-        const V3 v = v3((c & 1) ? q.hi0 : q.lo0, q.k, (c & 2) ? q.hi1 : q.lo1);
-#else
-        V3 v = v3(0.f);
-        v.set(q.kax, q.k);
-        v.set(q.a0, (c & 1) ? q.hi0 : q.lo0);
-        v.set(q.a1, (c & 2) ? q.hi1 : q.lo1);
-#endif
-        if (!light_point_far(v, p, w, sgn, m)) return false;
-      }
+      if (!rect_light_far(L, p, w, sgn, ps)) return false;
     } else if (L.kind == LIGHT_SPHERE) {
       const DSphere sp = S.spheres[L.idx];
       const V3 c = v3(sp.c0[0], sp.c0[1], sp.c0[2]);
@@ -2386,8 +2407,9 @@
   return true;
 }
 
-SRR_D int skip_mixture(const SceneView& S, const DiffSetup& me, bool dead, bool& pend, int& tries, uint64_t& lcg,
-                       V3& ndir, float& pdf, int max_rounds = 1 << 30) {
+template <bool ONE>
+SRR_D int skip_mixture(const SceneView& S, const DLightR& L0, const DiffSetup& me, bool dead, bool& pend, int& tries,
+                       uint64_t& lcg, V3& ndir, float& pdf, int max_rounds = 1 << 30) {
   int rounds = 0;
   while (rounds < max_rounds && __ballot(pend)) {
     if (pend) {
@@ -2407,7 +2429,7 @@
       Rng rr{s, 0};
       Bsdf f = bsdf_of(me);
       V3 nd;
-      const float pv = mixture_attempt(S, f, me.p, rr, nd);
+      const float pv = mixture_attempt<ONE>(S, L0, f, me.p, rr, nd);
       lcg = rr.lcg;
       tries = t + 1;
       if (pv != 0 || tries >= kMixtureGuard) {
@@ -2630,15 +2652,15 @@
 
 SRR_D V3 hit_emitted(const SceneView& S, int mat, V3 rdir, V3 hpt, V3 nrm, float hu, float hv) {
   if (mat < 0) return v3(0.f);
-  const DMat& M = S.mats[mat];
-  if (M.kind == MAT_DIFFUSE_LIGHT && dot(nrm, rdir) < 0.0) return tex_value(S, M.tex, hu, hv, hpt);
+  const DMatR& M = S.mats[mat];
+  if (M.kind == MAT_DIFFUSE_LIGHT && dot(nrm, rdir) < 0.0) return mat_color(S, M, hu, hv, hpt);
   return v3(0.f);
 }
 
 constexpr uint32_t kSpecMark = 0x7f800001u;
 
 template <int F>
-SRR_D void scatter(const SceneView& S, const DMat& M, V3 rdir, float rtime, V3 hpt, V3 nrm, float hu, float hv,
+SRR_D void scatter(const SceneView& S, const DMatR& M, V3 rdir, float rtime, V3 hpt, V3 nrm, float hu, float hv,
                    Rng& rng, float4& rec, bool& spec, V3& ndir, float& ntime, int* attempts = nullptr) {
   ntime = 0.0f;
   if (F == FAM_SPEC) {
@@ -2680,12 +2702,12 @@
       ndir = (r01 < reflect_prob) ? reflected : refracted;
     } else {
       ndir = random_in_unit_sphere(rng);
-      atten = tex_value(S, M.tex, hu, hv, hpt);
+      atten = mat_color(S, M, hu, hv, hpt);
     }
     rec = make_float4(atten.x, atten.y, atten.z, __uint_as_float(kSpecMark));
     spec = true;
   } else {
-    V3 atten = tex_value(S, M.tex, hu, hv, hpt);
+    V3 atten = mat_color(S, M, hu, hv, hpt);
     Bsdf f;
     f.kind = (F == FAM_BECK) ? (int)MAT_BECKMANN : M.kind;
     f.n = nrm;
@@ -2736,7 +2758,7 @@
   }
   float4 hp = ntl(&P.hit_p[p]), hn = ntl(&P.hit_n[p]);
   V3 hpt = v3(hp.x, hp.y, hp.z), nrm = v3(hn.x, hn.y, hn.z);
-  const DMat M = S.mats[mat];
+  const DMatR M = S.mats[mat];
   Rng rng{ntl(&P.lcg[p]), ntl(&P.pcg[p])};
   V3 ndir;
   float ntime;
@@ -2858,9 +2880,9 @@
       S.stris = (const DStandaloneTri*)(b + S.world_off[4]);
       S.meshes = (const DMesh*)(b + S.world_off[5]);
       S.media = (const DMedium*)(b + S.world_off[6]);
-      S.mats = (const DMat*)(b + S.world_off[7]);
+      S.mats = (const DMatR*)(b + S.world_off[7]);
       S.texs = (const DTex*)(b + S.world_off[8]);
-      S.lights = (const DLight*)(b + S.world_off[9]);
+      S.lights = (const DLightR*)(b + S.world_off[9]);
     }
     return S;
   };
@@ -3101,8 +3123,8 @@
         if (fam == FAM_TERM) {
           C = hit_emitted(S, h.mat, r.d, h.p, h.n, h.u, h.v);
         } else if ((!ALLFAM || fam == FAM_DIFF) && S.n_lights > 0) {
-          const DMat M = S.mats[h.mat];
-          d_atten = tex_value(S, M.tex, h.u, h.v, h.p);
+          const DMatR M = S.mats[h.mat];
+          d_atten = mat_color(S, M, h.u, h.v, h.p);
           Bsdf f;
           f.kind = M.kind;
           f.n = h.n;
@@ -3118,7 +3140,7 @@
           done = false;
           if (TIMED) fam_dt[2] = __builtin_amdgcn_s_memtime() - tq;
         } else {
-          const DMat M = S.mats[h.mat];
+          const DMatR M = S.mats[h.mat];
           float4 rec;
           bool sp;
           V3 nd;
@@ -3159,12 +3181,18 @@
       const SceneView S = view();
       const uint64_t tc = TIMED ? __builtin_amdgcn_s_memtime() : 0;
       int rounds = 0;
-      if (SRR_MIXTURE_SKIP == 1) {
-        rounds = skip_mixture(S, ds, d_dead, pend, d_tries, rng.lcg, d_dir, d_pdf);
-      } else {
-        if (SRR_MIXTURE_SKIP == 2) rounds = skip_mixture(S, ds, d_dead, pend, d_tries, rng.lcg, d_dir, d_pdf, 1);
-        if (__ballot(pend)) rounds += coop_mixture(S, ds, pend, d_tries, rng.lcg, d_dir, d_pdf, paths_args()->W.deep_tries);
-      }
+      const auto mixture = [&](auto one, const DLightR& L0) {
+        constexpr bool ONE = decltype(one)::value;
+        if (SRR_MIXTURE_SKIP == 1) {
+          rounds = skip_mixture<ONE>(S, L0, ds, d_dead, pend, d_tries, rng.lcg, d_dir, d_pdf);
+        } else {
+          if (SRR_MIXTURE_SKIP == 2) rounds = skip_mixture<ONE>(S, L0, ds, d_dead, pend, d_tries, rng.lcg, d_dir, d_pdf, 1);
+          if (__ballot(pend))
+            rounds += coop_mixture<ONE>(S, L0, ds, pend, d_tries, rng.lcg, d_dir, d_pdf, paths_args()->W.deep_tries);
+        }
+      };
+      if (S.light_one) mixture(std::true_type{}, uni(S.lights[0]));
+      else mixture(std::false_type{}, DLightR{});
       if (TIMED) {
         tp[6] += __builtin_amdgcn_s_memtime() - tc;
         tp[7] += rounds;
@@ -3496,7 +3524,8 @@
 }
 
 enum KatKind : int { KAT_ERF, KAT_BECK11, KAT_BECK_DIST, KAT_BECK_PDF, KAT_COSINE, KAT_ORENNAYAR, KAT_DIELECTRIC,
-                     KAT_METAL, KAT_TRIANGLE, KAT_AABB, KAT_SQRT, KAT_CAMERA, KAT_LIGHTS, KAT_LIGHT_LIST };
+                     KAT_METAL, KAT_TRIANGLE, KAT_AABB, KAT_SQRT, KAT_CAMERA, KAT_LIGHTS, KAT_LIGHT_LIST,
+                     KAT_LIGHT_ROW };
 
 SRR_D V3 kat3(const float* p) { return v3(p[0], p[1], p[2]); }
 SRR_D void kat_put3(float* p, V3 v) { p[0] = v.x, p[1] = v.y, p[2] = v.z; }
@@ -3576,7 +3605,7 @@
     }
     case KAT_DIELECTRIC:
     case KAT_METAL: {
-      DMat M{};
+      DMatR M{};
       if (kind == KAT_DIELECTRIC) {
         M.kind = MAT_DIELECTRIC;
         M.p[0] = r[0];
@@ -3659,6 +3688,14 @@
       kat_put_lcg(r + 13, rng.lcg);
       break;
     }
+    case KAT_LIGHT_ROW: {
+      const float lo0 = r[0], hi0 = r[1], lo1 = r[2], hi1 = r[3], k = r[4];
+      r[5] = (hi0 - lo0) * (hi1 - lo1);
+      r[6] = fmaxf(fmaxf(fmaxf(fabsf(lo0), fabsf(hi0)), fmaxf(fabsf(lo1), fabsf(hi1))), fabsf(k));
+      r[7] = a[0];
+      r[8] = a[1];
+      break;
+    }
     case KAT_AABB: {
       const V3 d = kat3(r + 9);
       r[14] = slab(make_float4(r[0], r[1], r[2], 0), make_float4(r[3], r[4], r[5], 0), kat3(r + 6),
diff --git a/simple-raytracing-render_amd/csrc/renderer.cpp b/simple-raytracing-render_amd/csrc/renderer.cpp
--- a/simple-raytracing-render_amd/csrc/renderer.cpp
+++ b/simple-raytracing-render_amd/csrc/renderer.cpp
@@ -1,6 +1,7 @@
 #include "renderer.h"
 
 #include "multi.h"
+#include "resolved.h"
 
 #include <algorithm>
 #include <chrono>
@@ -48,7 +49,7 @@
   RCHK(hipSetDevice(device));
   std::vector<void*>& K = r->scene_bufs;
   DObj* objs; DXform* xf; DSphere* sph; DRect* rct; DStandaloneTri* st; DMesh* me; float* nodes; float* n4;
-  float* tp; TriShade* ts; DMedium* md; DMat* mt; DTex* tx; uint8_t* im; float* pr; int32_t* pp; DLight* li;
+  float* tp; TriShade* ts; DMedium* md; DMatR* mt; DTex* tx; uint8_t* im; float* pr; int32_t* pp; DLightR* li;
   DCamera* cm;
   DObvh* ob;
   DObvhChild* oc;
@@ -88,12 +89,14 @@
   RCHK(upload(&oc, F.obvh_children, K));
   RCHK(upload(&sg, F.sgroups, K));
   RCHK(upload(&sgi, F.sg_items, K));
-  RCHK(upload(&mt, F.mats, K));
+  const std::vector<DLightR> lights_r = resolve_lights(F.lights, F.rects);
+  const std::vector<DMatR> mats_r = resolve_mats(F.mats, F.texs);
+  RCHK(upload(&mt, mats_r, K));
   RCHK(upload(&tx, F.texs, K));
   RCHK(upload(&im, F.images, K));
   RCHK(upload(&pr, F.perlin_ranvec, K));
   RCHK(upload(&pp, F.perlin_perm, K));
-  RCHK(upload(&li, F.lights, K));
+  RCHK(upload(&li, lights_r, K));
   RCHK(upload(&cm, cam, K));
   std::vector<uint8_t> blob;
   int off[10];
@@ -109,9 +112,9 @@
   put(4, F.stris.data(), F.stris.size() * sizeof(DStandaloneTri));
   put(5, F.meshes.data(), F.meshes.size() * sizeof(DMesh));
   put(6, F.media.data(), F.media.size() * sizeof(DMedium));
-  put(7, F.mats.data(), F.mats.size() * sizeof(DMat));
+  put(7, mats_r.data(), mats_r.size() * sizeof(DMatR));
   put(8, F.texs.data(), F.texs.size() * sizeof(DTex));
-  put(9, F.lights.data(), F.lights.size() * sizeof(DLight));
+  put(9, lights_r.data(), lights_r.size() * sizeof(DLightR));
   uint8_t* wb;
   RCHK(upload(&wb, blob, K));
   SceneView& V = r->view;
@@ -168,6 +171,8 @@
   V.lights = li;
   V.n_lights = (int)F.lights.size();
   V.light_weight = V.n_lights > 0 ? (float)(1.0 / V.n_lights) : 0.f;
+  V.light_one = V.n_lights == 1 && lights_r[0].kind == LIGHT_XZRECT;
+  V.light_draws = common_light_draws(lights_r);
   V.cam = cm;
   r->has_meshes = !F.meshes.empty() || !F.obvhs.empty();
   r->diffuse_only = true;
diff --git a/simple-raytracing-render_amd/csrc/resolved.h b/simple-raytracing-render_amd/csrc/resolved.h
--- /dev/null
+++ b/simple-raytracing-render_amd/csrc/resolved.h
@@ -0,0 +1,58 @@
+#pragma once
+#include <cmath>
+#include <vector>
+
+#include "device_scene.h"
+
+namespace srr {
+
+inline DLightR resolve_light(const DLight& L, const std::vector<DRect>& rects) {
+  DLightR r{};
+  r.kind = L.kind;
+  r.idx = L.idx;
+  r.draws = L.kind == LIGHT_NONE ? 0 : 2;
+  if (L.kind == LIGHT_XZRECT) {
+    const DRect& q = rects[L.idx];
+    r.lo0 = q.lo0;
+    r.hi0 = q.hi0;
+    r.lo1 = q.lo1;
+    r.hi1 = q.hi1;
+    r.k = q.k;
+    const volatile float d0 = q.hi0 - q.lo0, d1 = q.hi1 - q.lo1;
+    r.area = d0 * d1;
+    r.mabs = std::fmax(std::fmax(std::fmax(std::fabs(q.lo0), std::fabs(q.hi0)), std::fmax(std::fabs(q.lo1), std::fabs(q.hi1))),
+                       std::fabs(q.k));
+  }
+  return r;
+}
+
+inline std::vector<DLightR> resolve_lights(const std::vector<DLight>& lights, const std::vector<DRect>& rects) {
+  std::vector<DLightR> out;
+  for (const DLight& L : lights) out.push_back(resolve_light(L, rects));
+  return out;
+}
+
+inline int common_light_draws(const std::vector<DLightR>& lights) {
+  int d = lights.empty() ? 2 : lights[0].draws;
+  for (const DLightR& L : lights)
+    if (L.draws != d) return -1;
+  return d;
+}
+
+inline std::vector<DMatR> resolve_mats(const std::vector<DMat>& mats, const std::vector<DTex>& texs) {
+  std::vector<DMatR> out;
+  for (const DMat& m : mats) {
+    DMatR r{};
+    r.kind = m.kind;
+    r.tex = m.tex;
+    for (int k = 0; k < 4; ++k) r.p[k] = m.p[k];
+    if (m.tex >= 0 && m.tex < (int)texs.size() && texs[m.tex].kind == TEX_CONST) {
+      for (int k = 0; k < 3; ++k) r.c[k] = texs[m.tex].c[k];
+      r.c_const = 1;
+    }
+    out.push_back(r);
+  }
+  return out;
+}
+
+}
```
